# peterzjx/DeepHall

Hardware: AMD Instinct MI355X
Metric: local-energies/sec + MCMC walker-steps/sec, N=6 2Q=15, 1/2/4/8 GPUs (higher is better)
Workload: dtype f32; 1 GPU; VMC iteration (mcmc_step 10 MH moves + local energy + stats all-reduce), nspins=[6, 0] flux=15, Psiformer 4x64 heads, 2 layers, 1 det; walkers_per_gpu=4096, global_batch=4096, parallelism=walker-dp1, walker_groups_per_gpu=1, gemm_arithmetic=x6all

## Files before the change

### deephall_amd/_lib.py

```python

from __future__ import annotations

import ctypes as C
import os
from pathlib import Path

LIB_PATH = Path(__file__).resolve().parent / "_lib" / "libdeephall_amd.so"

DH_NSTATS = 16
STAT_NAMES = [
    "energy_re",
    "energy_im",
    "clipped_re",
    "clipped_im",
    "ere2",
    "kinetic_re",
    "kinetic_im",
    "potential",
    "angular_momentum_z",
    "angular_momentum_z_square",
    "angular_momentum_square",
    "pmove",
    "nvalid",
    "clipped_lz2",
    "clipped_lz",
    "clipped_l2",
]

EXPORTS = [
    "dh_create",
    "dh_create_cf",
    "dh_destroy",
    "dh_last_error",
    "dh_version",
    "dh_param_layout",
    "dh_set_params",
    "dh_workspace_bytes",
    "dh_set_gemm_mode",
    "dh_logpsi",
    "dh_mcmc_step",
    "dh_local_energy",
    "dh_energy_stats",
    "dh_loss_diff",
    "dh_init_walkers",
    "dh_potential",
    "dh_histograms",
    "dh_monopole_orbitals",
    "dh_mh_init",
    "dh_mh_propose",
    "dh_mh_accept",
    "dh_kinetic_from_derivatives",
    "dh_debug_trunk",
    "dh_debug_gemm",
    "dh_debug_gemm_ln",
    "dh_debug_gemm_x6_ln",
    "dh_debug_chain_x6",
    "dh_debug_gemm_lnch",
    "dh_debug_set_lnch_form",
    "dh_debug_x6_plane_rows",
    "dh_debug_split_planes",
    "dh_debug_gemm_x6",
    "dh_debug_gemm_x6_choice",
    "dh_debug_route",
    "dh_ref_layout",
    "dh_set_params_ref",
    "dh_vjp_workspace_bytes",
    "dh_logpsi_vjp",
    "dh_grad_cotangent",
    "dh_adam_update",
    "dh_profile_enable",
    "dh_profile_read",
    "dh_debug_f_offset",
    "dh_debug_env_leaf",
    "dh_kfac_layout",
    "dh_kfac_workspace_bytes",
    "dh_kfac_vjp",
    "dh_kfac_step",
    "dh_ntk_workspace_bytes",
    "dh_ntk_tile_walkers",
    "dh_ntk",
    "dh_ntk_part",
    "dh_ntk_mirror",
    "dh_ntk_owner",
    "dh_minsr_matrix_workspace_bytes",
    "dh_minsr_matrix",
    "dh_ntk_jvp_workspace_bytes",
    "dh_ntk_jvp",
    "dh_fidelity_partial",
    "dh_fidelity_residual",
]

DH_NFID = 5


PROF_KINDS = ["gemm", "attention", "layernorm", "input", "det_value", "det_energy", "mcmc",
              "gemm_ch", "attention_ch", "layernorm_ch", "input_ch", "layer1_ch"]


class DhConfig(C.Structure):
    _fields_ = [
        ("struct_size", C.c_uint32),
        ("n_up", C.c_int),
        ("n_dn", C.c_int),
        ("flux", C.c_int),
        ("radius", C.c_float),
        ("interaction_strength", C.c_float),
        ("interaction_type", C.c_int),
        ("num_heads", C.c_int),
        ("heads_dim", C.c_int),
        ("num_layers", C.c_int),
        ("ndets", C.c_int),
        ("orbital_type", C.c_int),
        ("network_type", C.c_int),
        ("excitation_lz", C.c_float),
        ("cf_flux", C.c_int),
    ]

    def __init__(self, *args, **kw):
        super().__init__(*args, **kw)
        self.struct_size = C.sizeof(DhConfig)


_lib = None


def load(path: Path | str | None = None):
    global _lib
    if _lib is not None:
        return _lib
    p = Path(path) if path else Path(os.environ.get("DH_LIB_PATH") or LIB_PATH)
    if not p.exists():
        raise RuntimeError(
            f"deephall_amd HIP library not found at {p}. Build it with "
            "`python -c 'import __graft_entry__ as g; g.build()'` (no CPU fallback exists)."
        )
    lib = C.CDLL(str(p))
    vp, sz, i32, u64, i64 = C.c_void_p, C.c_size_t, C.c_int, C.c_uint64, C.c_int64
    lib.dh_create.argtypes = [C.POINTER(DhConfig), C.POINTER(vp)]
    lib.dh_create.restype = i32
    lib.dh_create_cf.argtypes = [C.POINTER(DhConfig), C.POINTER(C.c_int), i32, C.POINTER(vp)]
    lib.dh_create_cf.restype = i32
    lib.dh_destroy.argtypes = [vp]
    lib.dh_destroy.restype = None
    lib.dh_last_error.restype = C.c_char_p
    lib.dh_version.restype = C.c_char_p
    lib.dh_param_layout.argtypes = [vp, C.POINTER(sz), i32]
    lib.dh_param_layout.restype = i32
    lib.dh_set_params.argtypes = [vp, vp, sz, vp]
    lib.dh_set_params.restype = i32
    lib.dh_workspace_bytes.argtypes = [vp, i32, i32]
    lib.dh_workspace_bytes.restype = sz
    lib.dh_set_gemm_mode.argtypes = [vp, i32]
    lib.dh_set_gemm_mode.restype = i32
    lib.dh_logpsi.argtypes = [vp, vp, i32, vp, vp, sz, vp]
    lib.dh_logpsi.restype = i32
    lib.dh_mcmc_step.argtypes = [vp, vp, vp, vp, i32, i32, C.c_float, u64, u64, i64, vp, vp, sz, vp]
    lib.dh_mcmc_step.restype = i32
    lib.dh_local_energy.argtypes = [vp, vp, i32, vp, vp, vp, sz, vp]
    lib.dh_local_energy.restype = i32
    lib.dh_energy_stats.argtypes = [vp, vp, vp, vp, i32, i32, i32, vp, vp]
    lib.dh_energy_stats.restype = i32
    f32 = C.c_float
    lib.dh_loss_diff.argtypes = [vp, vp, vp, i32, vp, f32, f32, f32, vp, vp, vp]
    lib.dh_loss_diff.restype = i32
    lib.dh_init_walkers.argtypes = [vp, vp, i32, u64, i64, vp]
    lib.dh_init_walkers.restype = i32
    lib.dh_potential.argtypes = [vp, vp, i32, vp, vp]
    lib.dh_potential.restype = i32
    lib.dh_histograms.argtypes = [vp, i32, i32, i32, i32, vp, vp, vp]
    lib.dh_histograms.restype = i32
    lib.dh_monopole_orbitals.argtypes = [vp, i32, i32, vp, vp]
    lib.dh_monopole_orbitals.restype = i32
    lib.dh_debug_trunk.argtypes = [vp, vp, i32, i32, vp, sz, vp]
    lib.dh_debug_trunk.restype = i32
    lib.dh_debug_f_offset.argtypes = [vp, i32, i32]
    lib.dh_debug_f_offset.restype = sz
    lib.dh_debug_env_leaf.argtypes = [vp, i32, i32, i32, vp, vp]
    lib.dh_debug_env_leaf.restype = i32
    lib.dh_debug_gemm.argtypes = [i32, vp, i32, vp, i32, vp, vp, i32, vp, i32, i32, i32, i32, i32, vp]
    lib.dh_debug_gemm.restype = i32
    lib.dh_debug_gemm_ln.argtypes = [i32, i32, vp, i32, vp, i32, vp, vp, vp, i32, i32, vp]
    lib.dh_debug_gemm_ln.restype = i32
    lib.dh_debug_gemm_x6_ln.argtypes = [i32, i32, vp, i32, vp, i32, vp, vp, vp, i32, i32, vp]
    lib.dh_debug_gemm_x6_ln.restype = i32
    lib.dh_debug_chain_x6.argtypes = [vp, vp, i32, vp, vp, vp, i32, vp, vp, vp, i32, vp, i32, vp, i32, vp, i32, vp]
    lib.dh_debug_chain_x6.restype = i32
    lib.dh_debug_gemm_lnch.argtypes = [i32, i32, vp, vp, i32, vp, vp, vp, vp, i32, vp]
    lib.dh_debug_gemm_lnch.restype = i32
    lib.dh_debug_set_lnch_form.argtypes = [i32]
    lib.dh_debug_set_lnch_form.restype = i32
    lib.dh_debug_x6_plane_rows.argtypes = [i32]
    lib.dh_debug_x6_plane_rows.restype = i32
    lib.dh_debug_split_planes.argtypes = [vp, i32, i32, i32, vp, vp]
    lib.dh_debug_split_planes.restype = i32
    lib.dh_debug_gemm_x6.argtypes = [i32, vp, i32, vp, i32, vp, vp, i32, vp, i32, i32, i32, i32, i32, vp]
    lib.dh_debug_gemm_x6.restype = i32
    lib.dh_debug_gemm_x6_choice.argtypes = [i32, i32]
    lib.dh_debug_gemm_x6_choice.restype = i32
    lib.dh_debug_route.argtypes = [vp, i32, i32, C.POINTER(i32), i32]
    lib.dh_debug_route.restype = i32
    lib.dh_ref_layout.argtypes = [vp, C.POINTER(sz), i32]
    lib.dh_ref_layout.restype = i32
    lib.dh_set_params_ref.argtypes = [vp, vp, sz, vp]
    lib.dh_set_params_ref.restype = i32
    lib.dh_vjp_workspace_bytes.argtypes = [vp, i32]
    lib.dh_vjp_workspace_bytes.restype = sz
    lib.dh_logpsi_vjp.argtypes = [vp, vp, i32, vp, vp, vp, vp, sz, vp]
    lib.dh_logpsi_vjp.restype = i32
    lib.dh_kfac_layout.argtypes = [vp, C.POINTER(sz), i32]
    lib.dh_kfac_layout.restype = i32
    lib.dh_kfac_workspace_bytes.argtypes = [vp, i32]
    lib.dh_kfac_workspace_bytes.restype = sz
    lib.dh_kfac_vjp.argtypes = [vp, vp, i32, vp, vp, vp, vp, vp, sz, vp]
    lib.dh_kfac_vjp.restype = i32
    lib.dh_kfac_step.argtypes = [vp, vp, vp, f32, f32, vp, vp, f32, f32, f32, vp, vp, vp, sz, vp]
    lib.dh_kfac_step.restype = i32
    lib.dh_ntk_workspace_bytes.argtypes = [vp, i32]
    lib.dh_ntk_workspace_bytes.restype = sz
    lib.dh_ntk_tile_walkers.argtypes = [vp]
    lib.dh_ntk_tile_walkers.restype = i32
    lib.dh_ntk.argtypes = [vp, vp, i32, vp, vp, vp, vp, sz, vp]
    lib.dh_ntk.restype = i32
    lib.dh_ntk_part.argtypes = [vp, vp, i32, vp, vp, vp, vp, sz, i32, i32, vp]
    lib.dh_ntk_part.restype = i32
    lib.dh_ntk_mirror.argtypes = [vp, i32, vp]
    lib.dh_ntk_mirror.restype = i32
    lib.dh_ntk_owner.argtypes = [vp, i32, i32]
    lib.dh_ntk_owner.restype = i32
    lib.dh_minsr_matrix_workspace_bytes.argtypes = [i32]
    lib.dh_minsr_matrix_workspace_bytes.restype = sz
    lib.dh_minsr_matrix.argtypes = [vp, vp, i32, C.c_double, vp, vp, sz, vp]
    lib.dh_minsr_matrix.restype = i32
    lib.dh_ntk_jvp_workspace_bytes.argtypes = [vp, i32]
    lib.dh_ntk_jvp_workspace_bytes.restype = sz
    lib.dh_ntk_jvp.argtypes = [vp, vp, i32, vp, vp, vp, vp, vp, vp, sz, i32, i32, vp]
    lib.dh_ntk_jvp.restype = i32
    lib.dh_fidelity_partial.argtypes = [vp, vp, i32, vp, vp]
    lib.dh_fidelity_partial.restype = i32
    lib.dh_fidelity_residual.argtypes = [vp, vp, i32, vp, vp, vp]
    lib.dh_fidelity_residual.restype = i32
    lib.dh_grad_cotangent.argtypes = [vp, vp, i32, i32, vp, vp]
    lib.dh_grad_cotangent.restype = i32
    lib.dh_adam_update.argtypes = [vp, vp, vp, vp, sz, f32, f32, f32, f32, i32, vp]
    lib.dh_adam_update.restype = i32
    lib.dh_mh_init.argtypes = [vp, vp, vp, i32, vp]
    lib.dh_mh_init.restype = i32
    lib.dh_mh_propose.argtypes = [vp, vp, i32, i32, f32, u64, u64, i64, vp, vp]
    lib.dh_mh_propose.restype = i32
    lib.dh_mh_accept.argtypes = [vp, vp, vp, vp, vp, i32, i32, u64, u64, i64, vp, vp]
    lib.dh_mh_accept.restype = i32
    lib.dh_kinetic_from_derivatives.argtypes = [vp, vp, vp, i32, i32, C.c_double, C.c_double, vp, vp, vp]
    lib.dh_kinetic_from_derivatives.restype = i32
    lib.dh_profile_enable.argtypes = [vp, i32]
    lib.dh_profile_enable.restype = i32
    lib.dh_profile_read.argtypes = [vp, C.POINTER(C.c_double), i32]
    lib.dh_profile_read.restype = i32
    _lib = lib
    return lib


def check(rc: int):
    if rc != 0:
        msg = load().dh_last_error().decode(errors="replace")
        raise RuntimeError(f"deephall_amd error {rc}: {msg}")
```

### deephall_amd/csrc/api.cpp

```cpp
#include <hip/hip_runtime.h>

#include <cmath>
#include <cstdio>
#include <cstring>
#include <string>
#include <vector>

#include "dh_internal.h"

using namespace dh;

namespace {
thread_local std::string g_err;

int fail(int code, const std::string& msg) {
  g_err = msg;
  return code;
}

#define HIP_TRY(expr)                                                                       \
  do {                                                                                      \
    hipError_t e_ = (expr);                                                                 \
    if (e_ != hipSuccess) return fail(DH_EHIP, std::string(#expr ": ") + hipGetErrorString(e_)); \
  } while (0)
// ... 661 lines not shown
  launch_copy2d(ref(R.jas(0)), 1, pk(so + 2), 1, 1, 1, st);
  launch_copy2d(ref(R.jas(1)), 1, pk(so + 2) + 1, 1, 1, 1, st);
  if (d.L > 0) launch_small_gemm(4, 3 * D, D, pk(0), D, 0, pk(1), 3 * D, 0, pk(so + 3), 3 * D, 0, st);
}

}

extern "C" {

int dh_set_params(dh_handle* h, const float* params, size_t count, void* stream) {
  if (h && h->analytic()) return count == 0 ? DH_OK : fail(DH_EINVAL, "the Laughlin wavefunction has no parameters");
  if (!h || !params) return fail(DH_EINVAL, "null argument");
  if (count != h->offsets.back()) return fail(DH_EINVAL, "parameter count mismatch");
  if (int rc = ensure_param_buffers(h)) return rc;
  HIP_TRY(hipMemcpyAsync(h->params, params, count * sizeof(float), hipMemcpyDeviceToDevice, (hipStream_t)stream));
  assign_packed(h);
  if (int rc = derive_weights(h, (hipStream_t)stream)) return rc;
  h->params_set = true;
  h->ref_set = false;
  return DH_OK;
}

int dh_ref_layout(const dh_handle* h, size_t* offsets, int n) {
  if (!h) return fail(DH_EINVAL, "null handle");
  const int nseg = (int)h->ref_offsets.size() - 1;
  for (int i = 0; i < n && i <= nseg; ++i) offsets[i] = h->ref_offsets[i];
  return nseg;
}

int dh_set_params_ref(dh_handle* h, const float* ref, size_t count, void* stream) {
  if (h && h->analytic()) return count == 0 ? DH_OK : fail(DH_EINVAL, "the Laughlin wavefunction has no parameters");
  if (!h || !ref) return fail(DH_EINVAL, "null argument");
  if (count != h->ref_offsets.back()) return fail(DH_EINVAL, "reference parameter count mismatch");
  if (int rc = ensure_param_buffers(h)) return rc;
  if (!h->ref) HIP_TRY(hipMalloc(&h->ref, count * sizeof(float)));
  hipStream_t st = (hipStream_t)stream;
  HIP_TRY(hipMemcpyAsync(h->ref, ref, count * sizeof(float), hipMemcpyDeviceToDevice, st));
  pack_from_ref(h, st);
  HIP_TRY(hipGetLastError());
  assign_packed(h);
  if (int rc = derive_weights(h, st)) return rc;
  h->params_set = true;
  h->ref_set = true;
  return DH_OK;
}

int dh_set_gemm_mode(dh_handle* h, int mode) {
  if (!h) return fail(DH_EINVAL, "null handle");
  if (mode != DH_GEMM_F32 && mode != DH_GEMM_X6 && mode != DH_GEMM_X6_ALL && mode != DH_GEMM_X6_ALL_UNFUSED)
    return fail(DH_EINVAL, "bad GEMM mode");
  h->gemm_mode = mode;
  return DH_OK;
}

size_t dh_workspace_bytes(const dh_handle* h, int batch, int op) {
  if (!h || batch < 1) return 0;
  return carve(h->d, h->gemm_mode, batch, op == 1 ? h->d.C : 1, nullptr).total_bytes;
}

}

namespace {

void dense_gemm(int family, const float* X, int ldx, const float* W, const float* Wt, const uint16_t* Wp, int ldw,
                const float* bias, const float* Res, int ldr, float* Y, int ldy, int rows, int ncols, int K, int C,
                hipStream_t s) {
  if (family == GEMM_X6)
    launch_gemm_x6(X, ldx, Wp, x6_plane_rows(ncols), bias, Res, ldr, Y, ldy, rows, ncols, K, C, s);
  else if (family == GEMM_F32_NT)
    launch_gemm_nt(X, ldx, Wt, K, bias, Res, ldr, Y, ldy, rows, ncols, K, C, s);
  else
    launch_gemm(X, ldx, W, ldw, bias, Res, ldr, Y, ldy, rows, ncols, K, C, s);
}

struct Trunk {
  dh_handle* h;
  const Dims& d;
  const Params& P;
  const Work& w;
  hipStream_t s;
  const int nw, C, rows;
  const TrunkRoute r;
  const bool keep_h;
  const int D = d.D, KO = ofeat_k(d);
  const int ch = C > 1 ? PK_CH : 0;
  const double R = rows, DD = D, f4 = 4.0;

  void gemm(const float* X, int ldx, const float* W, const float* Wt, const uint16_t* Wp, int ldw, const float* bias,
            const float* Res, int ldr, float* Y, int ldy, int ncols, int K) const {
    PROF(PK_GEMM + ch, 2.0 * R * ncols * K, f4 * (R * K + (double)K * ncols + R * ncols * (Res ? 2 : 1)));
    dense_gemm(r.family, X, ldx, W, Wt, Wp, ldw, bias, Res, ldr, Y, ldy, rows, ncols, K, C, s);
  }
  X6Feat h0_feat(int l) const { return (r.h0_epilogue && l == 0) ? X6Feat{P.W0, w.geo, d.N, d.n_up} : X6Feat{}; }

  void layer_chain(int l, bool attn) const {
    const LayerParams& lp = P.layer[l];
    const bool last = l + 1 == d.L;
    const int n3 = last ? d.orb_cols : 3 * D;
    PROF(PK_GEMM, 2.0 * R * DD * (2.0 * DD + n3), f4 * (2.0 * R * DD + R * n3 + 2.0 * DD * DD + DD * n3));
    X6Feat feat = h0_feat(l);
    if (attn) {
      feat.W0qkv = P.W0qkv;
      feat.bqkv = lp.bqkv;
      feat.Mqk = P.Mqk;
      feat.L1V = P.L1VP;
      feat.L1B = P.L1BP;
    }
    launch_chain_x6(w.o, attn ? P.UP : lp.WolP, x6_plane_rows(D), lp.bol, lp.ln1, lp.WmP, x6_plane_rows(D), lp.bm,
                    lp.ln2, last ? P.WorbP : P.layer[l + 1].WqkvP, x6_plane_rows(n3),
                    last ? P.borb : P.layer[l + 1].bqkv, n3, last ? w.F : w.qkv, last ? d.ld_orb : 3 * D, w.h, rows,
                    feat, s, !last || keep_h);
  }
  void layer_ln_epilogue(int l) const {
    const LayerParams& lp = P.layer[l];
    const bool x6 = r.family == GEMM_X6;
    {
      PROF(PK_GEMM, 2.0 * R * DD * DD, f4 * (3.0 * R * DD + DD * DD));
      if (x6)
        launch_gemm_x6_ln(w.o, D, lp.WolP, x6_plane_rows(D), lp.bol, lp.ln1, w.h, rows, D, 0, 0, s, h0_feat(l));
      else
        launch_gemm_ln(w.o, D, lp.WolT, D, lp.bol, lp.ln1, w.h, rows, D, 0, 0, s);
    }
    PROF(PK_GEMM, 2.0 * R * DD * DD, f4 * (2.0 * R * DD + DD * DD));
    if (x6)
      launch_gemm_x6_ln(w.h, D, lp.WmP, x6_plane_rows(D), lp.bm, lp.ln2, w.h, rows, D, 1, 0, s);
    else
      launch_gemm_ln(w.h, D, lp.WmT, D, lp.bm, lp.ln2, w.h, rows, D, 1, 0, s);
  }
  void layer_lnch(int l) const {
    const LayerParams& lp = P.layer[l];
    {
      const bool of = r.ofeat && l == 0;
      const double KK = of ? KO : DD;
      PROF(PK_GEMM + PK_CH, 2.0 * R * DD * KK, f4 * (R * KK + 2.0 * R * DD + DD * KK));
      launch_gemm_lnch(d.N, w.o, of ? P.UP : lp.WolP, x6_plane_rows(D), lp.bol, lp.ln1, w.geo, w.h, nw * d.N, 0, s,
                       (r.h0_epilogue && l == 0) ? P.W0 : nullptr, d.n_up, of ? KO : D);
    }
    PROF(PK_GEMM + PK_CH, 2.0 * R * DD * DD, f4 * (3.0 * R * DD + DD * DD));
    launch_gemm_lnch(d.N, w.h, lp.WmP, x6_plane_rows(D), lp.bm, lp.ln2, w.geo, w.h, nw * d.N, 1, s);
  }
  void layer_lnch_whole() const {
    const LayerParams& lp = P.layer[0];
    PROF(PK_L1CH, 2.0 * R * DD * 3.0 * KO, f4 * (R * KO + R * DD));
    launch_gemm_lnch(d.N, w.o, P.UP, x6_plane_rows(D), lp.bol, lp.ln2, w.geo, w.h, nw * d.N, 2, s, P.W0, d.n_up, KO,
                     P.L1VP, P.L1BP);
  }
  void layer_l1ch() const {
    const LayerParams& lp = P.layer[0];
    PROF(PK_L1CH, 2.0 * R * DD * (24.0 + 27.0), f4 * (R * KO + R * DD));
    launch_layer1_ch(d, w.o, P.UT, P.L1VT, P.W0, lp.bol, lp.ln1, lp.ln2, w.geo, w.h, nw, s);
  }
  void layer_separate(int l) const {
    const LayerParams& lp = P.layer[l];
    const bool lf = r.h0_epilogue && l == 0;
    if (r.ofeat && l == 0)
      gemm(w.o, KO, nullptr, P.UT, P.UP, KO, lp.bol, lf ? nullptr : w.h, D, w.t, D, D, KO);
    else
      gemm(w.o, D, lp.Wol, lp.WolT, lp.WolP, D, lp.bol, lf ? nullptr : w.h, D, w.t, D, D, D);
    {
      PROF(PK_LN + ch, 0.0, f4 * R * 2.0 * DD);
      launch_layernorm(d, w.t, nullptr, lp.ln1, w.geo, w.h, nw, C, 0, s, lf ? P.W0 : nullptr);
    }
    gemm(w.h, D, lp.Wm, lp.WmT, lp.WmP, D, lp.bm, nullptr, 0, w.o, D, D, D);
    PROF(PK_LN + ch, 0.0, f4 * R * 3.0 * DD);
    launch_layernorm(d, nullptr, w.o, lp.ln2, w.geo, w.h, nw, C, 1, s);
  }

  int run(const float* x, bool geo_ready) const {
    if (!(geo_ready && r.input_skip)) {
      const bool wq = r.input_qkv;
      PROF(PK_INPUT + ch, 8.0 * R * DD * (wq ? 4 : 1), f4 * R * DD * (wq ? 4 : 1));
      launch_input(d, x, P.W0, wq ? P.W0qkv : nullptr, wq ? P.layer[0].bqkv : nullptr, r.input_h ? w.h : nullptr,
                   wq ? w.qkv : nullptr, w.geo, nw, C, s);
    }
    for (int l = 0; l < d.L; ++l) {
      const LayerParams& lp = P.layer[l];
      const int form = l == 0 ? r.form0 : r.form1;
      if (l > 0 && r.qkv_gemm)
        gemm(w.h, D, lp.Wqkv, lp.WqkvT, lp.WqkvP, 3 * D, lp.bqkv, nullptr, 0, w.qkv, 3 * D, 3 * D, D);
      if (form != LF_CHAIN_ATTN) {
        const bool f = r.attn_feat && l == 0;
        PROF(PK_ATTN + ch, 0.0, f4 * R * (f ? 1.0 : 4.0) * DD);
        launch_attention(d, w.qkv, w.geo, w.o, nw, C, s, f ? P.W0qkv : nullptr, f ? lp.bqkv : nullptr,
                         f ? P.Mqk : nullptr);
      }
      switch (form) {
        case LF_CHAIN:
        case LF_CHAIN_ATTN: layer_chain(l, form == LF_CHAIN_ATTN); break;
        case LF_LN_EPILOGUE: layer_ln_epilogue(l); break;
        case LF_LNCH_WHOLE: layer_lnch_whole(); break;
        case LF_LNCH_PAIR: layer_lnch(l); break;
        case LF_L1CH: layer_l1ch(); break;
        default: layer_separate(l); break;
      }
    }
    if (r.orbital == ORB_GEMM)
      gemm(w.h, D, P.Worb, P.WorbT, P.WorbP, d.ld_orb, P.borb, nullptr, 0, w.F, d.ld_orb, d.orb_cols, D);
    return check_launch();
  }
};

int run_trunk(dh_handle* h, const float* x, int nw, int C, const Work& w, hipStream_t s, bool geo_ready = false,
              bool keep_h = false) {
  return Trunk{h, h->d, h->p, w, s, nw, C, nw * h->d.N * C, w.route, keep_h}.run(x, geo_ready);
}

int launch_trial(dh_handle* h, const float* x, float* logpsi, float* e_l, float* obs, int nw, hipStream_t s) {
  if (!h->expo && !h->expo_host.empty()) {
    HIP_TRY(hipMalloc(&h->expo, h->expo_host.size() * sizeof(int)));
    HIP_TRY(hipMemcpy(h->expo, h->expo_host.data(), h->expo_host.size() * sizeof(int), hipMemcpyHostToDevice));
  }
  PROF(e_l ? PK_DET_ENERGY : PK_DET_VALUE, 0.0, e_l ? 48.0 * nw : 8.0 * nw * h->d.N);
  if (h->state == dh_handle::PFAFFIAN)
    launch_pfaffian(h->d, x, h->cfg.cf_flux, logpsi, e_l, obs, nw, s);
  else if (h->state == dh_handle::JAIN)
    launch_cf(h->d, x, h->expo, h->cf_dense, logpsi, e_l, obs, nw, s);
  else
    launch_laughlin(h->d, x, h->expo, logpsi, e_l, obs, nw, s);
  return check_launch();
}

int value_pass(dh_handle* h, const float* x, int nw, const Work& w, float* logpsi, hipStream_t s,
               bool geo_ready = false, const McmcEpi& epi = McmcEpi{}) {
  if (h->analytic()) return launch_trial(h, x, logpsi, nullptr, nullptr, nw, s);
  if (int rc = run_trunk(h, x, nw, 1, w, s, geo_ready)) return rc;
  {
    PROF(PK_DET_VALUE, 0.0, 4.0 * nw * h->d.N * h->d.ld_orb);
    launch_det_value(h->d, w.F, x, h->p.jastrow, h->norm, logpsi, nw, s, epi);
  }
  return check_launch();
}

int check_common(dh_handle* h, const void* x, int B, void* ws, size_t ws_bytes, size_t need) {
  if (!h) return fail(DH_EINVAL, "null handle");
  if (!h->params_set) return fail(DH_ESTATE, "parameters not set");
  if (!x || B < 1) return fail(DH_EINVAL, "bad walkers");
  if (!ws || ws_bytes < need) return fail(DH_ENOMEM, "workspace too small");
  return DH_OK;
}

}

extern "C" {

int dh_logpsi(dh_handle* h, const float* x, int B, float* logpsi, void* ws, size_t ws_bytes, void* stream) {
  const size_t need = h ? dh_workspace_bytes(h, B, 0) : 0;
  if (int rc = check_common(h, x, B, ws, ws_bytes, need)) return rc;
  if (!logpsi) return fail(DH_EINVAL, "null output");
  hipStream_t s = (hipStream_t)stream;
  Work w = carve(h->d, h->gemm_mode, B, 1, ws);
  return value_pass(h, x, B, w, logpsi, s);
}

int dh_mcmc_step(dh_handle* h, float* x, float* lp, int32_t* n_accept, int B, int steps, float width, uint64_t seed,
                 uint64_t counter, int64_t walker_offset, const float* noise, void* ws, size_t ws_bytes,
                 void* stream) {
  const size_t need = h ? dh_workspace_bytes(h, B, 0) : 0;
  if (int rc = check_common(h, x, B, ws, ws_bytes, need)) return rc;
  if (!lp || !n_accept || steps < 0) return fail(DH_EINVAL, "bad MCMC arguments");
  hipStream_t s = (hipStream_t)stream;
  const Dims& d = h->d;
  Work w = carve(d, h->gemm_mode, B, 1, ws);
  if (int rc = value_pass(h, x, B, w, w.logpsi, s)) return rc;
  launch_lp_from_logpsi(w.logpsi, lp, n_accept, B, s);
  const size_t nstride = (size_t)B * (2 * d.N + 1);
  const bool geo = !h->analytic();
  const bool fuse = geo;
  for (int st = 0; st < steps; ++st) {
    const float* nz = noise ? noise + st * nstride : nullptr;
    const uint64_t step = counter + (uint64_t)st;
    if (!fuse || st == 0) {
      PROF(PK_MCMC, 0.0, 16.0 * B * d.N);
      if (st == 0)
        launch_propose(d, x, w.x2, B, width, seed, step, walker_offset, nz, 0, s, geo ? w.geo : nullptr);
      else
        launch_accept_propose(d, x, w.x2, geo ? w.geo : nullptr, lp, w.logpsi, n_accept, B, width, seed, step - 1,
                              walker_offset, noise ? noise + (st - 1) * nstride : nullptr, nz, s);
    }
    McmcEpi epi{};
    if (fuse) {
      epi.on = 1;
      epi.propose = st + 1 < steps;
      epi.x = x;
      epi.x2 = w.x2;
      epi.geo = w.geo;
      epi.lp = lp;
      epi.nacc = n_accept;
      epi.width = width;
      epi.seed = seed;
      epi.step = step;
      epi.woff = walker_offset;
      epi.noise = nz;
      epi.noise2 = (noise && st + 1 < steps) ? noise + (st + 1) * nstride : nullptr;
    }
    if (int rc = value_pass(h, w.x2, B, w, w.logpsi, s, geo, epi)) return rc;
  }
  if (steps > 0 && !fuse) {
    PROF(PK_MCMC, 0.0, 16.0 * B * d.N);
    launch_accept(d, x, w.x2, lp, w.logpsi, n_accept, B, seed, counter + (uint64_t)(steps - 1), walker_offset,
                  noise ? noise + (steps - 1) * nstride : nullptr, 0, s);
  }
  return check_launch();
}

int dh_local_energy(dh_handle* h, const float* x, int B, float* e_l, float* obs, void* ws, size_t ws_bytes,
                    void* stream) {
  const size_t need1 = h ? dh_workspace_bytes(h, 1, 1) : 0;
// ... 785 lines not shown
    launch_small_gemm(D + 1, D, D + 1, stats + K.slots[L.A_o].off, D + 1, 0, Wt, D, 0, T, D, 0, s);
    launch_small_gemm(D, D, D + 1, Wt, D, 1, T, D, 0, stats + K.slots[L.A_Wl].off, D, 0, s);
    launch_small_gemm(D, D, D, ref(RS.lay(l, RWl)), D, 0, stats + K.slots[L.G_T].off, D, 0, T, D, 0, s);
    launch_small_gemm(D, D, D, T, D, 0, ref(RS.lay(l, RWl)), D, 1, stats + K.slots[L.G_out].off, D, 0, s);
  }
  launch_kfac_generic(w.fgrad, K.dev.gen, stats + K.nmat, 1.f / (float)B, s);
  return check_launch();
}

int dh_kfac_step(dh_handle* h, float* raw, const float* stats, float ema, float weight, const float* grad,
                 float* params, float lr, float damping, float norm_constraint, float* pgrad, double* info, void* ws,
                 size_t ws_bytes, void* stream) {
  if (!h || h->analytic()) return fail(DH_EINVAL, "KFAC needs a Psiformer handle");
  if (!raw || !grad || !pgrad || !info || !ws) return fail(DH_EINVAL, "null argument");
  if (!(weight > 0.f) || !(damping > 0.f)) return fail(DH_EINVAL, "KFAC needs weight > 0 and damping > 0");
  if (int rc = kfac_device(h)) return rc;
  const KfacHost& K = *h->kfac;
  const size_t nref = h->ref_offsets.back();
  if (ws_bytes < kfac_step_ws(&K)) return fail(DH_ENOMEM, "KFAC step workspace too small");
  hipStream_t s = (hipStream_t)stream;
  double* kbuf = reinterpret_cast<double*>(ws);
  double* tr = kbuf + align64(K.kbuf_doubles);
  double* tmp = tr + align64(K.slots.size());
  if (stats) launch_kfac_ema(raw, stats, K.nstats, ema, s);
  launch_kfac_invert(K.dev, raw, 1.0 / weight, std::sqrt((double)damping), tr, kbuf, tmp, s);
  launch_kfac_precondition(K.dev, grad, raw + K.nmat, 1.0 / weight, damping, kbuf, pgrad, nref, info, s);
  if (params) launch_kfac_update(params, pgrad, nref, info, lr, norm_constraint, s);
  return check_launch();
}

int dh_grad_cotangent(const float* diff, const float* nvalid, int B, int part, float* ct, void* stream) {
  if (!diff || !nvalid || !ct || B < 1 || (part != 0 && part != 1)) return fail(DH_EINVAL, "bad arguments");
  launch_cotangent(diff, nvalid, B, part, ct, (hipStream_t)stream);
  return check_launch();
}

int dh_adam_update(float* params, const float* grad, float* mu, float* nu, size_t n, float lr, float b1, float b2,
                   float eps, int step, void* stream) {
  if (!params || !grad || !mu || !nu || n == 0 || step < 0) return fail(DH_EINVAL, "bad arguments");
  launch_adam(params, grad, mu, nu, n, lr, b1, b2, eps, step, (hipStream_t)stream);
  return check_launch();
}

int dh_energy_stats(dh_handle* h, const float* e_l, const float* obs, const int32_t* n_accept, int B, int steps,
                    int penalties, float* out, void* stream) {
  (void)h;
  if (!e_l || !obs || !out) return fail(DH_EINVAL, "null argument");
  if (B < 1) return fail(DH_EINVAL, "dh_energy_stats needs B >= 1");
  launch_stats(e_l, obs, n_accept, B, steps, penalties, out, (hipStream_t)stream);
  return check_launch();
}

int dh_loss_diff(dh_handle* h, const float* e_l, const float* obs, int B, const float* stats, float lz_penalty,
                 float lz_center, float l2_penalty, float* diff, float* nvalid, void* stream) {
  (void)h;
  if (!e_l || !obs || !stats || !diff || !nvalid) return fail(DH_EINVAL, "null argument");
  if (B < 1) return fail(DH_EINVAL, "dh_loss_diff needs B >= 1");
  launch_loss_diff(e_l, obs, B, stats, lz_penalty, lz_center, l2_penalty, diff, nvalid, (hipStream_t)stream);
  return check_launch();
}

int dh_fidelity_partial(const float* logpsi, const float* logphi, int B, double* part, void* stream) {
  if (!logpsi || !logphi || !part) return fail(DH_EINVAL, "dh_fidelity_partial: null argument");
  if (B < 1) return fail(DH_EINVAL, "dh_fidelity_partial needs B >= 1");
  launch_fidelity_partial(logpsi, logphi, B, part, (hipStream_t)stream);
  return check_launch();
}

int dh_fidelity_residual(const float* logpsi, const float* logphi, int B, const double* total, float* resid,
                         void* stream) {
  if (!logpsi || !logphi || !total || !resid) return fail(DH_EINVAL, "dh_fidelity_residual: null argument");
  if (B < 1) return fail(DH_EINVAL, "dh_fidelity_residual needs B >= 1");
  launch_fidelity_residual(logpsi, logphi, B, total, resid, (hipStream_t)stream);
  return check_launch();
}

int dh_debug_trunk(dh_handle* h, const float* x, int B, int op, void* ws, size_t ws_bytes, void* stream) {
  const size_t need = h ? dh_workspace_bytes(h, B, op) : 0;
  if (int rc = check_common(h, x, B, ws, ws_bytes, need)) return rc;
  Work w = carve(h->d, h->gemm_mode, B, op == 1 ? h->d.C : 1, ws);
  if (!w.F)
    return fail(DH_EINVAL, "dh_debug_trunk: this config's local energy goes envelope first and maps no orbital "
                           "features F over the channel rows");
  return run_trunk(h, x, B, op == 1 ? h->d.C : 1, w, (hipStream_t)stream, false, true);
}

int dh_debug_env_leaf(const float* thph, int n, int M, int sq, float* out, void* stream) {
  if (!thph || !out || n < 1 || M < 1) return fail(DH_EINVAL, "bad env_leaf probe args");
  launch_env_leaf_probe(thph, n, M, sq, out, (hipStream_t)stream);
  return check_launch();
}

size_t dh_debug_f_offset(const dh_handle* h, int B, int op) {
  if (!h || B < 1) return (size_t)-1;
  Work w = carve(h->d, h->gemm_mode, B, op == 1 ? h->d.C : 1, reinterpret_cast<void*>(size_t(64)));
  if (!w.F) return (size_t)-1;
  return (size_t)(w.F - reinterpret_cast<float*>(size_t(64)));
}

int dh_debug_gemm(int variant, const float* X, int ldx, const float* W, int ldw, const float* bias, const float* R,
                  int ldr, float* Y, int ldy, int rows, int ncols, int K, int C, void* stream) {
  bool known = true;
  if (variant >= 100) {
    if (K % 32 != 0) return fail(DH_EINVAL, "NT GEMM needs K % 32 == 0");
    known = launch_gemm_nt_variant(variant - 100, X, ldx, W, ldw, bias, R, ldr, Y, ldy, rows, ncols, K, C,
                                   (hipStream_t)stream);
  } else {
    known = launch_gemm_variant(variant < 0 ? 0 : variant, X, ldx, W, ldw, bias, R, ldr, Y, ldy, rows, ncols, K, C,
                                (hipStream_t)stream);
  }
  if (!known) return fail(DH_EINVAL, "no GEMM variant " + std::to_string(variant));
  return check_launch();
}

int dh_debug_gemm_x6_choice(int rows, int ncols) { return gemm_x6_choose(rows, ncols); }

int dh_debug_route(const dh_handle* h, int B, int op, int* out, int n) {
  if (!h || h->analytic() || B < 1 || (n > 0 && !out)) return fail(DH_EINVAL, "bad route query");
  const int C = op == 1 ? h->d.C : 1;
  const TrunkRoute r = trunk_route(h->d, h->gemm_mode, C, B * h->d.N * C);
  if (n > 0) std::memcpy(out, &r, sizeof(int) * std::min(n, kTrunkRouteFields));
  return kTrunkRouteFields;
}

int dh_debug_x6_plane_rows(int ncols) { return x6_plane_rows(ncols); }

int dh_debug_split_planes(const float* Wt, int ldw, int ncols, int K, uint16_t* Wp, void* stream) {
  if (!Wt || !Wp || ncols < 1 || K < 1) return fail(DH_EINVAL, "bad split_planes args");
  launch_split_planes(Wt, ldw, ncols, K, Wp, (hipStream_t)stream);
  return check_launch();
}

int dh_debug_gemm_x6(int variant, const float* X, int ldx, const uint16_t* Wp, int ldp, const float* bias,
                     const float* R, int ldr, float* Y, int ldy, int rows, int ncols, int K, int C, void* stream) {
  if (!gemm_x6_supported(K) || ldp < x6_plane_rows(ncols)) return fail(DH_EINVAL, "bad gemm_x6 args");
  if (variant >= 10 && K > 256) return fail(DH_EINVAL, "persistent gemm_x6 needs K <= 256");
  if (variant < 0) variant = gemm_x6_choose(rows, ncols);
  if (!launch_gemm_x6_variant(variant, X, ldx, Wp, ldp, bias, R, ldr, Y, ldy, rows, ncols, K, C, (hipStream_t)stream))
    return fail(DH_EINVAL, "no gemm_x6 variant " + std::to_string(variant));
  return check_launch();
}

int dh_debug_gemm_x6_ln(int mode, int nw, const float* X, int ldx, const uint16_t* Wp, int ldp, const float* bias,
                        const float* ln, float* h, int rows, int K, void* stream) {
  if (!gemm_x6_supported(K) || K > 256 || ldp < x6_plane_rows(256) || rows < 1 || (mode != 0 && mode != 1))
    return fail(DH_EINVAL, "bad gemm_x6_ln args");
  if (!launch_gemm_x6_ln(X, ldx, Wp, ldp, bias, ln, h, rows, K, mode, nw, (hipStream_t)stream))
    return fail(DH_EINVAL, "no gemm_x6_ln form " + std::to_string(nw));
  return check_launch();
}

int dh_debug_chain_x6(const float* X1, const uint16_t* Wp1, int ldp1, const float* b1, const float* ln1,
                      const uint16_t* Wp2, int ldp2, const float* b2, const float* ln2, const uint16_t* Wp3,
                      int ldp3, const float* b3, int n3, float* Y3, int ldy3, float* h, int rows, void* stream) {
  if (!X1 || !Wp1 || !Wp2 || !b1 || !ln1 || !b2 || !ln2 || !h || rows < 1 || ldp1 < x6_plane_rows(256) ||
      ldp2 < x6_plane_rows(256) || (Wp3 && (!b3 || !Y3 || n3 < 1 || ldy3 < n3 || ldy3 % 4 || ldp3 < x6_plane_rows(n3))))
    return fail(DH_EINVAL, "bad chain_x6 args");
  launch_chain_x6(X1, Wp1, ldp1, b1, ln1, Wp2, ldp2, b2, ln2, Wp3, ldp3, b3, n3, Y3, ldy3, h, rows, X6Feat{},
                  (hipStream_t)stream);
  return check_launch();
}

int dh_debug_gemm_lnch(int N, int mode, const float* X, const uint16_t* Wp, int ldp, const float* bias,
                       const float* ln, const float* geo, float* h, int ne, void* stream) {
  if (!gemm_lnch_supported(N, 256) || (mode != 0 && mode != 1) || (mode == 0 && !X) || !Wp || !ln || !geo || !h ||
      ne < 1 || ldp < x6_plane_rows(256) || ne % N)
    return fail(DH_EINVAL, "bad gemm_lnch args");
  launch_gemm_lnch(N, mode == 0 ? X : h, Wp, ldp, bias, ln, geo, h, ne, mode, (hipStream_t)stream);
  return check_launch();
}

int dh_debug_set_lnch_form(int form) { return set_lnch_form(form); }

int dh_debug_gemm_ln(int mode, int bm, const float* X, int ldx, const float* Wt, int ldw, const float* bias,
                     const float* ln, float* h, int rows, int K, void* stream) {
  if (!gemm_ln_supported(256, K) || rows < 1 || (mode != 0 && mode != 1)) return fail(DH_EINVAL, "bad gemm_ln args");
  launch_gemm_ln(X, ldx, Wt, ldw, bias, ln, h, rows, K, mode, bm, (hipStream_t)stream);
  return check_launch();
}

int dh_profile_enable(dh_handle* h, int on) {
  if (!h) return fail(DH_EINVAL, "null handle");
  h->prof.on = on != 0;
  h->prof.used = 0;
  return DH_OK;
}

int dh_profile_read(dh_handle* h, double* out, int reset) {
  if (!h || !out) return fail(DH_EINVAL, "null argument");
  for (int i = 0; i < 4 * PK_TOTAL; ++i) out[i] = 0.0;
  for (size_t i = 0; i < h->prof.used; ++i) {
    ProfRec& r = h->prof.recs[i];
    HIP_TRY(hipEventSynchronize(r.b));
    float ms = 0.f;
    HIP_TRY(hipEventElapsedTime(&ms, r.a, r.b));
    out[4 * r.kind + 0] += 1.0;
    out[4 * r.kind + 1] += ms;
    out[4 * r.kind + 2] += r.flops;
    out[4 * r.kind + 3] += r.bytes;
  }
  if (reset) h->prof.used = 0;
  return PK_TOTAL;
}

int dh_potential(dh_handle* h, const float* x, int B, float* pe, void* stream) {
  if (!h || !x || !pe || B < 1) return fail(DH_EINVAL, "bad arguments");
  launch_potential(h->d, x, pe, B, (hipStream_t)stream);
  return check_launch();
}

int dh_histograms(const float* x, int B, int nelec, int density_bins, int pair_bins, float* density, float* pair,
                  void* stream) {
  if (!x || B < 1 || nelec < 1 || density_bins < 0 || pair_bins < 0 || density_bins + pair_bins < 1 ||
      density_bins + pair_bins > 8192 || (density_bins && !density) || (pair_bins && !pair))
    return fail(DH_EINVAL, "bad arguments");
  launch_histograms(x, B, nelec, density_bins, pair_bins, density, pair, (hipStream_t)stream);
  return check_launch();
}

int dh_monopole_orbitals(const float* points, int n, int flux, float* out, void* stream) {
  if (!points || !out || n < 1 || flux < 0 || flux > 126) return fail(DH_EINVAL, "bad arguments");
  launch_monopole_orbitals(points, n, flux, out, (hipStream_t)stream);
  return check_launch();
}


int dh_mh_init(const float* logpsi, float* lp, int32_t* n_accept, int B, void* stream) {
  if (!logpsi || !lp || !n_accept || B < 1) return fail(DH_EINVAL, "bad arguments");
  launch_lp_from_logpsi(logpsi, lp, n_accept, B, (hipStream_t)stream);
  return check_launch();
}

int dh_mh_propose(const float* x, float* x2, int B, int nelec, float width, uint64_t seed, uint64_t step,
                  int64_t walker_offset, const float* noise, void* stream) {
  if (!x || !x2 || B < 1 || nelec < 1 || x == x2) return fail(DH_EINVAL, "bad arguments");
  Dims d{};
  d.N = nelec;
  launch_propose(d, x, x2, B, width, seed, step, walker_offset, noise, 0, (hipStream_t)stream);
  return check_launch();
}

int dh_mh_accept(float* x, const float* x2, float* lp, const float* logpsi2, int32_t* n_accept, int B, int nelec,
                 uint64_t seed, uint64_t step, int64_t walker_offset, const float* noise, void* stream) {
  if (!x || !x2 || !lp || !logpsi2 || !n_accept || B < 1 || nelec < 1) return fail(DH_EINVAL, "bad arguments");
  Dims d{};
  d.N = nelec;
  launch_accept(d, x, x2, lp, logpsi2, n_accept, B, seed, step, walker_offset, noise, 0, (hipStream_t)stream);
  return check_launch();
}

int dh_kinetic_from_derivatives(const double* x, const double* grad, const double* hess, int B, int nelec, double Q,
                                double r, float* ke, float* mom, void* stream) {
  if (!x || !grad || !hess || !ke || !mom || B < 1 || nelec < 1 || !(r > 0.0) || Q < 0.0)
    return fail(DH_EINVAL, "bad arguments");
  if (kinetic_assembly_lds_bytes(nelec) > 64 * 1024) return fail(DH_EINVAL, "nelec > 256");
// ... 12 lines not shown
```

### deephall_amd/csrc/det.hip

```cpp
#include <cstdlib>
#include <type_traits>

#include "dh_internal.h"
#include "device_common.h"
#include "mcmc_common.h"

#ifndef DET_LU_REG
#define DET_LU_REG 0
#endif
#ifndef DET_WAVE_SQ
#define DET_WAVE_SQ 1
#endif
#ifndef DET_LEAF_SQ
#define DET_LEAF_SQ 1
#endif
#ifndef DET_GJ_REG
#define DET_GJ_REG 1
#endif
#ifndef DET_STAMP
#define DET_STAMP 0
#endif
#if DET_STAMP
constexpr int DET_STAMP_WG = 1024, DET_NSTAMP = 12;
__device__ unsigned long long g_det_stamp[2 * DET_STAMP_WG * DET_NSTAMP];
#define DET_T(slot, i)                                                                                       \
  do {                                                                                                      \
    if (threadIdx.x == 0 && blockIdx.x < DET_STAMP_WG)                                                       \
      g_det_stamp[((slot) * DET_STAMP_WG + blockIdx.x) * DET_NSTAMP + (i)] = __builtin_amdgcn_s_memtime();     \
  } while (0)
extern "C" int dh_debug_det_stamps(unsigned long long* out, int n) {
  n = n < 2 * DET_STAMP_WG * DET_NSTAMP ? n : 2 * DET_STAMP_WG * DET_NSTAMP;
  return hipMemcpyFromSymbol(out, HIP_SYMBOL(g_det_stamp), n * sizeof(unsigned long long)) == hipSuccess ? 0 : -1;
}
#else
#define DET_T(slot, i)
#endif

namespace dh {
namespace {

__device__ inline float ipow(float b, int e) { return e < 0 ? 0.f : (e == 0 ? 1.f : powf(b, (float)e)); }
__device__ inline float ipow_sq(float b, int e) {
  float r = 1.f;
  for (; e > 0; e >>= 1, b *= b)
    if (e & 1) r *= b;
  return r;
}

struct FView {
  const float* F;
  int ld, M, N, K;
  __device__ inline cf at(size_t row, int blk, int m, int j, int k) const {
    const size_t base = row * ld;
    const int MNK = M * N * K;
    const int off = m * N * K + j * K + k;
    return cf{F[base + (size_t)(blk * 2) * MNK + off], F[base + (size_t)(blk * 2 + 1) * MNK + off]};
  }
};

struct EnvLeaf {
  cf e0, dth, dph, lb, d2th;
};
__device__ __forceinline__ float env_gauge(float ct, int M) {
  return (float)(M - 1) * __builtin_rintf(64.f * ct) * (1.f / 128.f);
}
__device__ inline EnvLeaf env_leaf(float th, float ph, int p, int M, float norm, bool leaves, float gauge = 0.f,
                                   bool sq = false) {
  const int a = p, b = M - 1 - p;
  const float m = 0.5f * (float)(a - b) - gauge;
  float c, s;
  sincosf(0.5f * th, &s, &c);
  float sph, cph;
  sincosf(m * ph, &sph, &cph);
  const float R = sq ? ipow_sq(c, a) * ipow_sq(s, b) : ipow(c, a) * ipow(s, b);
  EnvLeaf L;
  L.e0 = cf{norm * R * cph, norm * R * sph};
  if (leaves) {
    const float fa = (float)a, fb = (float)b;
    auto pw = [sq](float x, int e) { return sq ? (e < 0 ? 0.f : ipow_sq(x, e)) : ipow(x, e); };
    const float R1 = 0.5f * (fb * pw(c, a + 1) * pw(s, b - 1) - fa * pw(c, a - 1) * pw(s, b + 1));
    const float R2 = 0.25f * (fb * (fb - 1.f) * pw(c, a + 2) * pw(s, b - 2) - fb * (fa + 1.f) * R -
                              fa * (fb + 1.f) * R + fa * (fa - 1.f) * pw(c, a - 2) * pw(s, b + 2));
    float st, ct;
    sincosf(th, &st, &ct);
    L.dth = cf{norm * R1 * cph, norm * R1 * sph};
    L.d2th = cf{norm * R2 * cph, norm * R2 * sph};
    L.dph = cf{-m * L.e0.im / st, m * L.e0.re / st};
    const float cot = ct / st;
    const float k2 = m * m / (st * st);
    L.lb = cf{L.d2th.re - k2 * L.e0.re + cot * L.dth.re, L.d2th.im - k2 * L.e0.im + cot * L.dth.im};
  }
  return L;
}

__device__ inline cf env_flow2(const cf& e0, const cf& dth, const cf& d2th, float m, float st, float ct, float sp,
                               float cp, int k) {
  const float cot = ct / st;
  const float ph_hat[3] = {-sp, cp, 0.f};
  const float th_hat[3] = {ct * cp, ct * sp, -st};
  const float thp[3] = {cp * cot, sp * cot, -1.f};
  const float dthp_dth[3] = {-cp / (st * st), -sp / (st * st), 0.f};
  const float dthp_dph[3] = {-sp * cot, cp * cot, 0.f};
  const float cs[3] = {cp, sp, 0.f};
  const float td = ph_hat[k];
  const float pd = -th_hat[k] / st;
  const float tdd = cs[k] * thp[k];
  const float pdd = -(dthp_dth[k] * td - dthp_dph[k] * thp[k]);
  cf r;
  r.re = d2th.re * td * td + 2.f * (-m * dth.im) * td * pd + (-m * m * e0.re) * pd * pd + dth.re * tdd +
         (-m * e0.im) * pdd;
  r.im = d2th.im * td * td + 2.f * (m * dth.re) * td * pd + (-m * m * e0.im) * pd * pd + dth.im * tdd +
         (m * e0.re) * pdd;
  return r;
}

__device__ inline void find_pivot(const cf* A, int lda, int N, int p, int* piv, int tid, int width) {
  if (tid < width) {
    const int lane = tid;
    float best = -1.f;
    int bi = N;
    for (int r = p + lane; r < N; r += width) {
      const float v = cabs1(A[r * lda + p]);
      if (v > best) {
        best = v;
        bi = r;
      }
    }
    for (int o = width >> 1; o > 0; o >>= 1) {
      const float ob = __shfl_xor(best, o, width);
      const int oi = __shfl_xor(bi, o, width);
      if (ob > best || (ob == best && oi < bi)) {
        best = ob;
        bi = oi;
      }
    }
    if (lane == 0) *piv = (bi < N) ? bi : p;
  }
}

__device__ __forceinline__ void eliminate(cf* A, int lda, int N, int ncol, bool gj, cf* fac, int* piv, cf* logdet,
                          int tid = threadIdx.x, int nt = blockDim.x, int width = 64) {
  if (tid == 0) *logdet = cf{0.f, 0.f};
  __syncthreads();
  for (int p = 0; p < N; ++p) {
    find_pivot(A, lda, N, p, piv, tid, width);
    __syncthreads();
    const int pr = *piv;
    if (pr != p) {
      for (int c = tid; c < ncol; c += nt) {
        const cf t = A[p * lda + c];
        A[p * lda + c] = A[pr * lda + c];
        A[pr * lda + c] = t;
      }
    }
    __syncthreads();
    const cf P = A[p * lda + p];
    if (tid == 0) {
      const float mag = sqrtf(P.re * P.re + P.im * P.im);
      logdet->re += logf(mag);
      logdet->im += atan2f(P.im, P.re) + (pr != p ? kPi : 0.f);
    }
    const cf Pinv = cdiv(cf{1.f, 0.f}, P);
    __syncthreads();
    if (gj) {
      for (int r = tid; r < N; r += nt) fac[r] = (r == p) ? cf{0.f, 0.f} : A[r * lda + p];
      for (int c = tid; c < ncol; c += nt) A[p * lda + c] = A[p * lda + c] * Pinv;
    } else {
      for (int r = tid; r < N; r += nt) fac[r] = (r > p) ? A[r * lda + p] * Pinv : cf{0.f, 0.f};
    }
    __syncthreads();
    const int r0 = gj ? 0 : p + 1;
    const int c0 = gj ? 0 : p;
    const int nr = N - r0, nc = ncol - c0;
    for (int idx = tid; idx < nr * nc; idx += nt) {
      const int r = r0 + idx / nc, c = c0 + idx % nc;
      if (r == p) continue;
      const cf f = fac[r];
      cf v = A[r * lda + c];
      const cf a = A[p * lda + c];
      v.re -= f.re * a.re - f.im * a.im;
      v.im -= f.re * a.im + f.im * a.re;
      A[r * lda + c] = v;
    }
    __syncthreads();
  }
}

template <int NMAX>
__device__ __forceinline__ cf gj_inverse_cols(cf (&col)[NMAX], int N) {
  auto is = [](int r, int q) __attribute__((always_inline)) {
    int m = r == q;
    asm volatile("" : "+v"(m));
    return m != 0;
  };
  auto pick = [&](int q) __attribute__((always_inline)) {
    cf v = col[0];
#pragma unroll
    for (int r = 1; r < NMAX; ++r)
      if (is(r, q)) v = col[r];
    return v;
  };
  float lre = 0.f, lim = 0.f;
  for (int p = 0; p < N; ++p) {
    float best = -1.f;
    int bi = N;
#pragma unroll
    for (int r = 0; r < NMAX; ++r) {
      if (r >= p && r < N) {
        const float v = cabs1(col[r]);
        if (v > best) {
          best = v;
          bi = r;
        }
      }
    }
    int pr = __shfl(bi, p, 64);
    pr = pr < N ? pr : p;
    if (pr != p) {
      const cf a = pick(p), b = pick(pr);
#pragma unroll
      for (int r = 0; r < NMAX; ++r) {
        if (is(r, p)) col[r] = b;
        if (is(r, pr)) col[r] = a;
      }
    }
    const cf mine = pick(p);
    const cf P{__shfl(mine.re, p, 64), __shfl(mine.im, p, 64)};
    const float mag = sqrtf(P.re * P.re + P.im * P.im);
    lre += logf(mag);
    lim += atan2f(P.im, P.re) + (pr != p ? kPi : 0.f);
    const cf rowp = mine * cdiv(cf{1.f, 0.f}, P);
#pragma unroll
    for (int r = 0; r < NMAX; ++r) {
      if (r < N) {
        const cf f{__shfl(col[r].re, p, 64), __shfl(col[r].im, p, 64)};
        cf v = col[r];
        v.re -= f.re * rowp.re - f.im * rowp.im;
        v.im -= f.re * rowp.im + f.im * rowp.re;
        col[r] = is(r, p) ? rowp : v;
      }
    }
  }
  return cf{lre, lim};
}

template <int NMAX>
__device__ __forceinline__ cf lu_logdet_cols(cf (&col)[NMAX], int N, int lane, int width) {
  auto is = [](int r, int q) __attribute__((always_inline)) {
    int m = r == q;
    asm volatile("" : "+v"(m));
    return m != 0;
  };
  auto pick = [&](int q) __attribute__((always_inline)) {
    cf v = col[0];
#pragma unroll
    for (int r = 1; r < NMAX; ++r)
      if (is(r, q)) v = col[r];
    return v;
  };
  float lre = 0.f, lim = 0.f;
  for (int p = 0; p < N; ++p) {
    float best = -1.f;
    int bi = N;
#pragma unroll
    for (int r = 0; r < NMAX; ++r) {
      if (r >= p && r < N) {
        const float v = cabs1(col[r]);
        if (v > best) {
          best = v;
          bi = r;
        }
      }
    }
    int pr = __shfl(bi, p, width);
    pr = pr < N ? pr : p;
    if (pr != p) {
      const cf a = pick(p), b = pick(pr);
#pragma unroll
      for (int r = 0; r < NMAX; ++r) {
        if (is(r, p)) col[r] = b;
        if (is(r, pr)) col[r] = a;
      }
    }
    const cf mine = pick(p);
    const cf P{__shfl(mine.re, p, width), __shfl(mine.im, p, width)};
    const float mag = sqrtf(P.re * P.re + P.im * P.im);
    lre += logf(mag);
    lim += atan2f(P.im, P.re) + (pr != p ? kPi : 0.f);
    const cf Pinv = cdiv(cf{1.f, 0.f}, P);
#pragma unroll
    for (int r = 0; r < NMAX; ++r) {
      if (r > p && r < N) {
#pragma clang fp contract(off)
        const cf c = col[r];
        const cf fl{c.re * Pinv.re - c.im * Pinv.im, __builtin_fmaf(c.im, Pinv.re, c.re * Pinv.im)};
        const cf f{__shfl(fl.re, p, width), __shfl(fl.im, p, width)};
        if (lane >= p) {
          const float tre = __builtin_fmaf(f.re, mine.re, -(f.im * mine.im));
          const float tim = __builtin_fmaf(f.im, mine.re, f.re * mine.im);
          col[r] = cf{c.re - tre, c.im - tim};
        }
      }
    }
  }
  return cf{lre, lim};
}

__device__ inline double jastrow_pair(double r, double al, double cst, double* f1, double* f2) {
  const double ar = al + r;
  *f1 = (cst * al * al) / (ar * ar);
  *f2 = -2.0 * (cst * al * al) / (ar * ar * ar);
  return -(cst * al * al) / ar;
}

template <int MGV, bool HW = false>
__global__ __launch_bounds__(64) void det_value_kernel(const float* __restrict__ Fp, int ldF, const float* x,
                                 const float* __restrict__ jas, const float* __restrict__ norm, float* __restrict__ logpsi,
                                 int N, int n_up, int M, int K, int nw, int per, McmcEpi epi) {
  static_assert(!HW || MGV == 0, "half-wave form: serial contraction only");
  extern __shared__ float sm_all[];
  const int half = HW ? (int)(threadIdx.x >> 5) : 0;
  float* sm_raw = sm_all + half * per;
  cf* E0 = reinterpret_cast<cf*>(sm_raw);
  cf* A = E0 + N * M;
  cf* fac = A + N * N;
  cf* ld = fac + N;
  cf* logdet = ld + K;
  int* piv = reinterpret_cast<int*>(logdet + 1);
  const int bw = HW ? 2 * (int)blockIdx.x + half : (int)blockIdx.x;
  const bool live = bw < nw;
  const int b = live ? bw : nw - 1;
  const int tid = HW ? (int)(threadIdx.x & 31) : (int)threadIdx.x, nt = HW ? 32 : 64, width = HW ? 32 : 64;
  double* cart = reinterpret_cast<double*>(piv + 2);
  DET_T(0, 0);
  for (int idx = tid; idx < N * M; idx += nt) {
    const int i = idx / M, p = idx % M;
    E0[idx] = env_leaf(x[2 * (b * N + i)], x[2 * (b * N + i) + 1], p, M, norm[p], false, 0.f, true).e0;
  }
  for (int i = tid; i < N; i += nt) {
    double st, ct, sp, cp;
    sincos((double)x[2 * (b * N + i)], &st, &ct);
    sincos((double)x[2 * (b * N + i) + 1], &sp, &cp);
    cart[3 * i] = st * cp;
    cart[3 * i + 1] = st * sp;
    cart[3 * i + 2] = ct;
  }
  __syncthreads();
  DET_T(0, 1);
  double Jw = 0.0;
  {
    const double ap = jas[0], aa = jas[1];
    for (int q = tid; q < N * N; q += nt) {
      const int i = q / N, j = q - (q / N) * N;
      if (j <= i) continue;
      const double dx = cart[3 * j] - cart[3 * i], dy = cart[3 * j + 1] - cart[3 * i + 1],
                   dz = cart[3 * j + 2] - cart[3 * i + 2];
      const double r = sqrt(dx * dx + dy * dy + dz * dz);
      const bool same = (i < n_up) == (j < n_up);
      double f1, f2;
      Jw += jastrow_pair(r, same ? ap : aa, same ? 0.25 : 0.5, &f1, &f2);
    }
    for (int o = width >> 1; o > 0; o >>= 1) Jw += __shfl_xor(Jw, o, width);
  }
  DET_T(0, 2);
  const int G = 64 / N, gj = tid % N, gg = tid / N, NK = N * K, MNK = M * NK;
  for (int k = 0; k < K; ++k) {
    if constexpr (MGV == 0) {
      for (int idx = tid; idx < N * N; idx += nt) {
        const int i = idx / N, j = idx % N;
        const int blk = (i >= n_up && n_up > 0) ? 1 : 0;
        const float* rp = Fp + ((size_t)b * N + i) * ldF + (size_t)blk * 2 * MNK + (size_t)j * K + k;
        cf acc{0.f, 0.f};
        for (int p0 = 0; p0 < M; p0 += 16) {
          float fr[16], fi[16];
#pragma unroll
          for (int q = 0; q < 16; ++q) {
            const size_t p = (size_t)min(p0 + q, M - 1);
            fr[q] = rp[p * NK];
            fi[q] = rp[(size_t)MNK + p * NK];
          }
#pragma unroll
          for (int q = 0; q < 16; ++q)
            if (p0 + q < M) cfma(acc, cf{fr[q], fi[q]}, E0[i * M + p0 + q]);
        }
        A[idx] = acc;
      }
    }
    if constexpr (MGV > 0) {
      constexpr int NF = 2 * (MGV > 0 ? MGV : 1);
      auto ldrow = [&](int i, float (&f)[NF]) __attribute__((always_inline)) {
        const int blk = (i >= n_up && n_up > 0) ? 1 : 0;
        const float* rp = Fp + ((size_t)b * N + i) * ldF + (size_t)blk * 2 * MNK + (size_t)gj * K + k;
#pragma unroll
        for (int u = 0; u < MGV; ++u) {
          const size_t m = (size_t)min(gg + G * u, M - 1);
          f[2 * u] = rp[m * NK];
          f[2 * u + 1] = rp[(size_t)MNK + m * NK];
        }
      };
      auto contract = [&](int i, const float (&f)[NF]) __attribute__((always_inline)) {
        cf acc{0.f, 0.f};
#pragma unroll
        for (int u = 0; u < MGV; ++u) {
          const int m = gg + G * u;
          const bool ok = gg < G && m < M;
          cfma(acc, cf{ok ? f[2 * u] : 0.f, ok ? f[2 * u + 1] : 0.f}, E0[i * M + min(m, M - 1)]);
        }
        float re = acc.re, im = acc.im;
        for (int q = 1; q < G; ++q) {
          re += __shfl(acc.re, gj + N * q, 64);
          im += __shfl(acc.im, gj + N * q, 64);
        }
        if (gg == 0) A[i * N + gj] = cf{re, im};
      };
      float fa[NF], fb[NF];
      if constexpr (MGV <= 24) {
        ldrow(0, fa);
        for (int i = 0; i < N; i += 2) {
          ldrow(min(i + 1, N - 1), fb);
          contract(i, fa);
          ldrow(min(i + 2, N - 1), fa);
          if (i + 1 < N) contract(i + 1, fb);
        }
      } else {
        for (int i = 0; i < N; ++i) {
          ldrow(i, fa);
          contract(i, fa);
        }
      }
    }
    __syncthreads();
    DET_T(0, 3);
    if (N <= 8 && DET_LU_REG) {
      cf col[8];
#pragma unroll
      for (int r = 0; r < 8; ++r) col[r] = (r < N && tid < N) ? A[r * N + tid] : cf{0.f, 0.f};
      const cf l = lu_logdet_cols<8>(col, N, tid, width);
      if (tid == 0) ld[k] = l;
    } else {
      eliminate(A, N, N, N, false, fac, piv, logdet, tid, nt, width);
      if (tid == 0) ld[k] = *logdet;
    }
    __syncthreads();
    DET_T(0, 4);
  }
  float* lpv = reinterpret_cast<float*>(cart + 3 * N);
  if (tid == 0 && live) {
    float lmax = -INFINITY;
    for (int k = 0; k < K; ++k) lmax = fmaxf(lmax, ld[k].re);
    float zr = 0.f, zi = 0.f;
    for (int k = 0; k < K; ++k) {
      const float mag = expf(ld[k].re - lmax);
      zr += mag * cosf(ld[k].im);
      zi += mag * sinf(ld[k].im);
    }
    float val_re = 0.5f * logf(zr * zr + zi * zi) + lmax;
    float val_im = atan2f(zi, zr);
    logpsi[2 * b] = val_re + (float)Jw;
    logpsi[2 * b + 1] = val_im;
    *lpv = val_re + (float)Jw;
  }
  DET_T(0, 5);
  if (!epi.on) return;
  __syncthreads();
  if (!live || tid >= N) return;
  const float lp2 = 2.f * *lpv;
  const bool cond = accept_one(lp2, epi.lp[b], b, N, epi.seed, epi.step, epi.woff, epi.noise);
  const int e = b * N + tid;
  float th = epi.x[2 * e], ph = epi.x[2 * e + 1];
  if (cond) {
    th = x[2 * e];
    ph = x[2 * e + 1];
    epi.x[2 * e] = th;
    epi.x[2 * e + 1] = ph;
    if (tid == 0) {
      epi.lp[b] = lp2;
      epi.nacc[b] += 1;
    }
  }
  if (epi.propose)
    propose_one(th, ph, epi.x2, epi.geo, e, b, tid, N, epi.width, epi.seed, epi.step + 1, epi.woff, epi.noise2);
  DET_T(0, 6);
}

#ifndef ENV_REG
#define ENV_REG 1
#endif
#ifndef ENV_SEG_RING
#define ENV_SEG_RING 4
#endif
constexpr int kEnvSegRing = ENV_SEG_RING;
__host__ __device__ constexpr int env_ring(int MG) { return (63 / (2 * MG) + 1) < 4 ? (63 / (2 * MG) + 1) : 4; }

template <int MG, bool WU = false, int SEG = 0>
__global__ __launch_bounds__(256) void env_contract_kernel(const float* __restrict__ Fp, int ldF,
                                                           const float* __restrict__ x,
                                                           const float* __restrict__ geo_g,
                                                           const float* __restrict__ norm, float* __restrict__ PhiC,
                                                           int nw, int N, int n_up, int M, int K, float Q) {
  static_assert(SEG == 0 || !WU, "segment DMA: four waves per electron");
  constexpr int Q2 = SEG ? 2 * SEG : 2 * MG, RING = SEG ? kEnvSegRing : env_ring(MG);
  static_assert((RING - 1) * Q2 <= 63, "vmcnt range");
  extern __shared__ float sm[];
  const int tid = threadIdx.x, lane = tid & 63, wv = tid >> 6;
  const int unit = WU ? blockIdx.x * 4 + wv : blockIdx.x;
  if (WU && unit >= nw * N) return;
  const int b = unit / N, i = unit - (unit / N) * N;
  const int T = 2 * N, C = 2 * N + 5;
  const int wsz = WU ? 20 * M + ((3 * T + 3) & ~3) + RING * Q2 * 64 : 0;
  cf* wt = reinterpret_cast<cf*>(sm + (size_t)wv * wsz);
  cf* part = wt + 10 * M;
  float* al = reinterpret_cast<float*>(WU ? part : part + 4 * C * N);
  float* ring = al + ((3 * T + 3) & ~3);
  const int G = 64 / N, j = lane % N, g = lane / N, S = WU ? G : 4 * G;
  const int MW = (M + 3) / 4;
  const int gg = SEG ? MW * wv + g : (WU ? g : G * wv + g);
  const int mend = SEG ? min(MW * (wv + 1), M) : M;
  const bool act = g < G;
  const int blk = (i >= n_up && n_up > 0) ? 1 : 0;
  const int NK = N * K, MNK = M * NK;
  auto gsum = [&](float v) __attribute__((always_inline)) {
    float r = v;
    for (int q = 1; q < G; ++q) r += __shfl(v, j + N * q, 64);
    return r;
  };
  auto gsumc = [&](cf v) __attribute__((always_inline)) { return cf{gsum(v.re), gsum(v.im)}; };
  const float* rowbase = Fp + ((size_t)(b * N + i) * C) * ldF + (size_t)blk * 2 * MNK + (size_t)j * K;
  const int SS = SEG ? G : S;
  auto mw = [&](int u) __attribute__((always_inline)) { return min(gg + SS * u, M - 1); };
  auto okm = [&](int u) __attribute__((always_inline)) { return act && gg + SS * u < mend; };
  const int segf = MW * N * K;
  float* wring = WU ? ring : ring + (size_t)wv * RING * (SEG ? 2 * segf : Q2 * 64);
  const uint32_t ring0 = (uint32_t)(size_t)((__attribute__((address_space(3))) char*)wring);
  const float* segbase = Fp + ((size_t)(b * N + i) * C) * ldF + (size_t)blk * 2 * MNK + (size_t)MW * wv * NK;
  const int segb = (mend - MW * wv) * NK * 4;
  auto issue = [&](int c, int kd) __attribute__((always_inline)) {
    if constexpr (SEG > 0) {
      (void)kd;
      const int slot = c % RING;
#pragma unroll
      for (int q = 0; q < 2 * SEG; ++q) {
        const int p = q / SEG, piece = q % SEG;
        const int byte = piece * 1024 + lane * 16;
        const char* src = reinterpret_cast<const char*>(segbase + (size_t)c * ldF + (p ? (size_t)MNK : 0)) + byte;
        const uint32_t dst = __builtin_amdgcn_readfirstlane(ring0 + (uint32_t)(slot * 2 * segf * 4 + p * segf * 4 + piece * 1024));
        if (byte < segb) {
          unsigned keep;
          asm volatile("s_mov_b32 %0, m0\n\ts_mov_b32 m0, %2\n\ts_nop 0\n\tglobal_load_lds_dwordx4 %1, off\n\ts_mov_b32 m0, %0"
                       : "=&s"(keep)
                       : "v"(src), "s"(dst)
                       : "memory");
        }
      }
      return;
    }
    const float* rp = rowbase + (size_t)c * ldF + kd;
    const int slot = c % RING;
#pragma unroll
    for (int q = 0; q < Q2; ++q) {
      const int u = q >> 1;
      const float* src = okm(u) ? rp + ((q & 1) ? (size_t)MNK : 0) + (size_t)(gg + S * u) * NK : rowbase;
      const uint32_t dst = __builtin_amdgcn_readfirstlane(ring0 + (uint32_t)((slot * Q2 + q) * 256));
      unsigned keep;
      asm volatile("s_mov_b32 %0, m0\n\ts_mov_b32 m0, %2\n\ts_nop 0\n\tglobal_load_lds_dword %1, off\n\ts_mov_b32 m0, %0"
                   : "=&s"(keep)
// ... 1343 lines not shown
      const int blk = (i >= n_up && n_up > 0) ? 1 : 0;
      const size_t row = (size_t)b * N + i;
      cf acc{0.f, 0.f};
      for (int p = 0; p < M; ++p) cfma(acc, F.at(row, blk, p, j, k), E0[i * M + p]);
      A[i * lda + j] = acc;
      if (lda > N) A[i * lda + N + j] = cf{i == j ? 1.f : 0.f, 0.f};
    }
    __syncthreads();
  };
  if (K > 1) {
    for (int k = 0; k < K; ++k) {
      build(k, N);
      eliminate(A, N, N, N, false, fac, piv, logdet);
      if (tid == 0) ld[k] = *logdet;
      __syncthreads();
    }
    if (tid == 0) {
      float lmax = -INFINITY;
      for (int k = 0; k < K; ++k) lmax = fmaxf(lmax, ld[k].re);
      cf z{0.f, 0.f};
      for (int k = 0; k < K; ++k) {
        const float mag = expf(ld[k].re - lmax);
        z += cf{mag * cosf(ld[k].im), mag * sinf(ld[k].im)};
      }
      for (int k = 0; k < K; ++k) {
        const float mag = expf(ld[k].re - lmax);
        wk[k] = cdiv(cf{mag * cosf(ld[k].im), mag * sinf(ld[k].im)}, z);
      }
    }
  } else if (tid == 0) {
    wk[0] = cf{1.f, 0.f};
  }
  __syncthreads();
  for (int k = 0; k < K; ++k) {
    build(k, 2 * N);
    eliminate(A, 2 * N, N, 2 * N, true, fac, piv, logdet);
    const cf w = wk[k];
    for (int idx = tid; idx < N * M * N; idx += nt) {
      const int i = idx / (M * N), rem = idx - i * (M * N), p = rem / N, j = rem - (rem / N) * N;
      const int blk = (i >= n_up && n_up > 0) ? 1 : 0;
      const cf f = w * A[j * 2 * N + N + i];
      const cf G{cr * f.re + ci * f.im, ci * f.re - cr * f.im};
      const cf e = E0[i * M + p];
      const cf v{G.re * e.re + G.im * e.im, G.im * e.re - G.re * e.im};
      const size_t rowoff = ((size_t)b * N + i) * ldF;
      const int off = p * N * K + j * K + k;
      dF[rowoff + (size_t)(blk * 2) * MNK + off] = v.re;
      dF[rowoff + (size_t)(blk * 2 + 1) * MNK + off] = v.im;
    }
    __syncthreads();
  }
}

__global__ void potential_kernel(const float* __restrict__ x, float* __restrict__ pe, int nw, int N, float Q,
                                 float radius, int interaction) {
  const int b = blockIdx.x * blockDim.x + threadIdx.x;
  if (b >= nw) return;
  double acc = 0.0;
  for (int i = 0; i < N; ++i) {
    const double ti = x[2 * (b * N + i)], pi_ = x[2 * (b * N + i) + 1];
    const double xi = sin(ti) * cos(pi_), yi = sin(ti) * sin(pi_), zi = cos(ti);
    for (int j = i + 1; j < N; ++j) {
      const double tj = x[2 * (b * N + j)], pj = x[2 * (b * N + j) + 1];
      const double u = xi * sin(tj) * cos(pj) + yi * sin(tj) * sin(pj) + zi * cos(tj);
      if (interaction == DH_INTERACTION_COULOMB)
        acc += 1.0 / sqrt(2.0 - 2.0 * u);
      else
        acc += 1.0 + ((double)Q + 1.0) / (double)Q * u;
    }
  }
  if (interaction == DH_INTERACTION_COULOMB) acc /= (double)radius;
  pe[b] = (float)acc;
}

}

void launch_potential(const Dims& d, const float* x, float* pe, int nw, hipStream_t s) {
  hipLaunchKernelGGL(potential_kernel, dim3((nw + 127) / 128), dim3(128), 0, s, x, pe, nw, d.N, d.Q, d.r,
                     d.interaction);
}

void launch_det_value(const Dims& d, const float* F, const float* x, const float* jastrow, const float* norm,
                      float* logpsi, int nw, hipStream_t s, const McmcEpi& epi) {
  const int per = (2 * d.N * d.M + 2 * d.N * d.N + 2 * d.N + 2 * d.K + 2 + 4 + 6 * d.N + 2 + 3 + 1) & ~3;
  auto go = [&](auto kern) {
    hipLaunchKernelGGL(kern, dim3(nw), dim3(64), (size_t)per * sizeof(float), s, F, d.ld_orb, x, jastrow, norm,
                       logpsi, d.N, d.n_up, d.M, d.K, nw, per, epi);
  };
  const int mgv = (d.M + 64 / d.N - 1) / (64 / d.N);
  if (mgv <= 2 && d.N * d.N <= 64) {
    hipLaunchKernelGGL((det_value_kernel<0, true>), dim3((nw + 1) / 2), dim3(64), (size_t)2 * per * sizeof(float), s, F,
                       d.ld_orb, x, jastrow, norm, logpsi, d.N, d.n_up, d.M, d.K, nw, per, epi);
  } else if (mgv <= 2)
    go(det_value_kernel<0>);
  else if (mgv <= 4)
    go(det_value_kernel<4>);
  else if (mgv <= 8)
    go(det_value_kernel<8>);
  else if (mgv <= 16)
    go(det_value_kernel<16>);
  else if (mgv <= 24)
    go(det_value_kernel<24>);
  else if (mgv <= 32)
    go(det_value_kernel<32>);
  else
    go(det_value_kernel<64>);
}

void launch_det_bwd(const Dims& d, const float* F, const float* x, const float* jastrow, const float* norm,
                    const float* ct, float* dF, float* jg, int nw, hipStream_t s) {
  const size_t bytes =
      (size_t)(2 * d.N * d.M + 4 * d.N * d.N + 2 * d.N + 4 * d.K + 2 + 4 + 6 * d.N + 2) * sizeof(float);
  ensure_smem(det_bwd_kernel, bytes);
  hipLaunchKernelGGL(det_bwd_kernel, dim3(nw), dim3(64), bytes, s, F, d.ld_orb, x, jastrow, norm, ct, dF, jg, d.N,
                     d.n_up, d.M, d.K, d.orb_cols);
}

bool det_precontract(const Dims& d) {
  const bool fits = 2 * d.K * d.N <= d.D && d.N <= 32 && d.M <= 16 * 4 * (64 / d.N) && d.M <= 128;
  return fits && !(det_staged(d.N, d.M, d.K) && 2 * d.M * d.N * d.K * d.N <= 8 * 256);
}

static int det_wave_nv(const Dims& d, bool& vec) {
  if (d.N > kDetWaveMaxN || !det_staged(d.N, d.M, d.K)) return 0;
  const int RW = 2 * d.M * d.N * d.K;
  vec = (RW % 4 == 0) && (d.ld_orb % 4 == 0);
  const int units = vec ? d.N * RW / 4 : d.N * RW;
  const int need = (units + 63) / 64;
  for (int v : (vec ? std::initializer_list<int>{1, 2, 3, 5, 8, 12} : std::initializer_list<int>{1, 2, 4, 8, 16}))
    if (need <= v) return v;
  return 0;
}

void launch_det_energy(const Dims& d, const float* F, const float* x, const float* geo, const float* jastrow,
                       const float* norm, float* e_l, float* obs, int nw, hipStream_t s, float* phic) {
  bool vec = false;
  const int nv = phic ? 0 : det_wave_nv(d, vec);
  if (nv > 0) {
    const size_t bytes = (size_t)det_wave_layout(d.N, d.M, d.K).total * sizeof(float);
    auto go = [&](auto kern) {
      ensure_smem(kern, bytes);
      hipLaunchKernelGGL(kern, dim3(nw), dim3(64), bytes, s, F, d.ld_orb, x, geo, jastrow, norm, e_l, obs, d.N, d.n_up,
                         d.M, d.K, d.Q, d.r, d.lambda, d.interaction);
    };
    if (vec) {
      switch (nv) {
        case 1: go(det_energy_wave_kernel<1, true>); break;
        case 2: go(det_energy_wave_kernel<2, true>); break;
        case 3: go(det_energy_wave_kernel<3, true>); break;
        case 5: go(det_energy_wave_kernel<5, true>); break;
        case 8: go(det_energy_wave_kernel<8, true>); break;
        default: go(det_energy_wave_kernel<12, true>); break;
      }
    } else {
      switch (nv) {
        case 1: go(det_energy_wave_kernel<1, false>); break;
        case 2: go(det_energy_wave_kernel<2, false>); break;
        case 4: go(det_energy_wave_kernel<4, false>); break;
        case 8: go(det_energy_wave_kernel<8, false>); break;
        default: go(det_energy_wave_kernel<16, false>); break;
      }
    }
    return;
  }
  const DetSmem L = det_layout(d.N, d.M, d.K, 4, phic != nullptr);
  const size_t bytes = (size_t)L.total * sizeof(float);
  auto go = [&](auto kern) {
    ensure_smem(kern, bytes);
    hipLaunchKernelGGL(kern, dim3(nw), dim3(256), bytes, s, F, d.ld_orb, x, geo, jastrow, norm, e_l, obs, d.N, d.n_up,
                       d.M, d.K, d.Q, d.r, d.lambda, d.interaction, (const float*)phic);
  };
  const int nrw = 2 * d.M * d.N * d.K * d.N;
  if (phic) {
// ... 335 lines not shown
```

### deephall_amd/csrc/dh_internal.h

```cpp
#pragma once
#include <algorithm>
#include <hip/hip_runtime.h>
#include <stdint.h>
#include <stddef.h>

#include "../../include/deephall_amd.h"

namespace dh {

struct Dims {
  int N, n_up, n_dn;
  int T;
  int C;
  int M;
  float Q, r;
  int H, dh, D, L, K;
  int NB;
  int orb_cols;
  int ld_orb;
  int interaction;
  float lambda;
  int sparse;
};
constexpr int kSparseFeatures = 8;
constexpr int kMqkStride = 32;

struct LayerParams {
  const float *Wqkv, *bqkv, *Wol, *bol, *ln1, *Wm, *bm, *ln2;
  const uint16_t *WqkvB, *WolB, *WmB;
  const float *WqkvBT, *WolBT, *WmBT;
  const float *WqkvT, *WolT, *WmT;
  const uint16_t *WqkvP, *WolP, *WmP;
};
struct Params {
  const float* W0;
  LayerParams layer[16];
  const float *Worb, *borb, *jastrow;
  const float* W0qkv;
  const float* WorbT;
  const uint16_t* WorbP;
  const uint16_t* WorbB;
  const float* WorbBT;
  const float* Mqk;
  const float* UT;
  const uint16_t* UP;
  const uint16_t *L1VP, *L1BP;
  const float* L1VT;
  const float* W2T;
  const uint16_t* W2P;
};
inline int ofeat_k(const Dims& d) { return (8 * d.H + 31) / 32 * 32; }

struct Pass {
  int nw;
  int C;
  int rows;
  int rows_pad;
};

enum GemmFamily : int { GEMM_F32_NN = 0, GEMM_F32_NT = 1, GEMM_X6 = 2 };
enum LayerForm : int {
  LF_SEPARATE = 0,
  LF_LN_EPILOGUE,
  LF_CHAIN,
  LF_CHAIN_ATTN,
  LF_LNCH_PAIR,
  LF_LNCH_WHOLE,
  LF_L1CH,
};
enum OrbitalMap : int { ORB_NONE = 0, ORB_GEMM = 1, ORB_IN_CHAIN = 2 };
enum DetStage : int { DET_VALUE = 0, DET_DIRECT = 1, DET_PRECONTRACT = 2, DET_ENV_FIRST = 3 };
struct TrunkRoute {
  int family;
  int input_h;
  int input_qkv;
  int input_skip;
  int form0, form1;
  int attn_feat;
  int h0_epilogue;
  int ofeat;
  int qkv_gemm;
  int orbital;
  int det;
};
constexpr int kTrunkRouteFields = 12;
static_assert(sizeof(TrunkRoute) == kTrunkRouteFields * sizeof(int), "dh_debug_route copies the fields as ints");
int gemm_family(const Dims& d, bool want_x6);
TrunkRoute trunk_route(const Dims& d, int gemm_mode, int C, int rows);

constexpr int kRowPad = 256;
constexpr int kWalkerRowPad = 768;
inline int round_up(int a, int b) { return (a + b - 1) / b * b; }

template <typename Kern>
inline void ensure_smem(Kern kernel, size_t bytes) {
  if (bytes > 65536)
    (void)hipFuncSetAttribute(reinterpret_cast<const void*>(kernel), hipFuncAttributeMaxDynamicSharedMemorySize,
                              (int)bytes);
}

void launch_gemm(const float* X, int ldx, const float* W, int ldw, const float* bias, const float* R, int ldr,
                 float* Y, int ldy, int rows, int ncols, int K, int C, hipStream_t s);
bool launch_gemm_variant(int v, const float* X, int ldx, const float* W, int ldw, const float* bias, const float* R,
                         int ldr, float* Y, int ldy, int rows, int ncols, int K, int C, hipStream_t s);
bool launch_gemm_nt_variant(int v, const float* X, int ldx, const float* Wt, int ldw, const float* bias,
                            const float* R, int ldr, float* Y, int ldy, int rows, int ncols, int K, int C,
                            hipStream_t s);
void launch_gemm_nt(const float* X, int ldx, const float* Wt, int ldw, const float* bias, const float* R, int ldr,
                    float* Y, int ldy, int rows, int ncols, int K, int C, hipStream_t s);
bool gemm_ln_supported(int D, int K);
void launch_gemm_ln(const float* X, int ldx, const float* Wt, int ldw, const float* bias, const float* ln, float* h,
                    int rows, int K, int mode, int bm, hipStream_t s);
int x6_plane_rows(int ncols);
void launch_split_planes(const float* Wt, int ldw, int ncols, int K, uint16_t* Wp, hipStream_t s);
bool gemm_x6_supported(int K);
enum X6Form : int {
  X6D_128x192 = 44,
  X6D_256x128 = 46,
  X6Q_256x128 = 52,
  X6Q_256x256 = 56,
  X6Q_256x192 = 57,
  X6Q_256x160 = 58,
  X6M_256x256 = 76,
  X6M_256x192 = 77,
};
int gemm_x6_choose(int rows, int ncols);
bool launch_gemm_x6_variant(int v, const float* X, int ldx, const uint16_t* Wp, int ldp, const float* bias,
                            const float* R, int ldr, float* Y, int ldy, int rows, int ncols, int K, int C,
                            hipStream_t s);
void launch_gemm_x6(const float* X, int ldx, const uint16_t* Wp, int ldp, const float* bias, const float* R, int ldr,
                    float* Y, int ldy, int rows, int ncols, int K, int C, hipStream_t s);
struct X6Feat {
  const float* W0 = nullptr;
  const float* geo = nullptr;
  int N = 1, n_up = 0;
  const float* W0qkv = nullptr;
  const float* bqkv = nullptr;
  const float* Mqk = nullptr;
  const uint16_t* L1V = nullptr;
  const uint16_t* L1B = nullptr;
};
bool launch_gemm_x6_ln(const float* X, int ldx, const uint16_t* Wp, int ldp, const float* bias, const float* ln,
                       float* h, int rows, int K, int mode, int nw, hipStream_t s, X6Feat feat = X6Feat{});
bool gemm_lnch_supported(int N, int D);
int set_lnch_form(int f);
void launch_gemm_lnch(int N, const float* X, const uint16_t* Wp, int ldp, const float* bias, const float* ln,
                      const float* geo, float* h, int ne, int mode, hipStream_t s,
                      const float* W0f = nullptr, int n_up = 0, int K = 256, const uint16_t* Wv = nullptr,
                      const uint16_t* Wb = nullptr);
void launch_l1_basis(const Dims& d, const float* W0, const float* UT, const float* bol, const float* ln1,
                     const float* Wm, const float* bm, float* BT, float* VT, hipStream_t s);
bool chain_attn_supported(int N, int H, int dh);
void launch_chain_x6(const float* X1, const uint16_t* Wp1, int ldp1, const float* b1, const float* ln1,
                     const uint16_t* Wp2, int ldp2, const float* b2, const float* ln2, const uint16_t* Wp3, int ldp3,
                     const float* b3, int n3, float* Y3, int ldy3, float* h, int rows, X6Feat feat, hipStream_t s,
                     bool store_h = true);
void launch_transpose(const float* src, int ld_src, int rows, int cols, float* dst, int ld_dst, hipStream_t s);

void launch_input(const Dims& d, const float* x, const float* W0, const float* W0qkv, const float* bqkv, float* h,
                  float* qkv, float* geo, int nw, int C, hipStream_t s);
void launch_propose(const Dims& d, const float* x, float* x2, int nw, float width, uint64_t seed, uint64_t step,
                    int64_t walker_offset, const float* noise, int noise_stride, hipStream_t s, float* geo = nullptr);
void launch_accept_propose(const Dims& d, float* x, float* x2, float* geo, float* lp, const float* logpsi2,
                           int32_t* n_acc, int nw, float width, uint64_t seed, uint64_t step, int64_t walker_offset,
                           const float* noise, const float* noise2, hipStream_t s);
void launch_init_walkers(const Dims& d, float* x, int nw, uint64_t seed, int64_t walker_offset, hipStream_t s);

bool attention_takes_features(const Dims& d, int C);
bool attention_mfma_supported(const Dims& d);
void launch_attention_mfma(const Dims& d, const float* qkv, const float* geo, float* o, int nw, hipStream_t s,
                           const float* W0qkv, const float* bqkv);
void launch_attention(const Dims& d, const float* qkv, const float* geo, float* o, int nw, int C, hipStream_t s,
                      const float* W0qkv = nullptr, const float* bqkv = nullptr, const float* Mqk = nullptr);
void launch_lowrank_qk(const Dims& d, const float* W0qkv, const float* bqkv, float* Mqk, hipStream_t s);
void launch_ofeat_weight(const Dims& d, const float* W0qkv, const float* bqkv, const float* Wol, float* UT,
                         hipStream_t s);

void launch_layernorm(const Dims& d, const float* X, const float* Z, const float* ln, const float* geo, float* h,
                      int nw, int C, int mode, hipStream_t s,
                      const float* W0f = nullptr);
bool layer1_ch_supported(const Dims& d);
void launch_layer1_ch(const Dims& d, const float* O, const float* UT, const float* VT, const float* W0f,
                      const float* bol, const float* ln1, const float* ln2, const float* geo, float* h, int nw,
                      hipStream_t s);

struct McmcEpi {
  int on = 0, propose = 0;
  float* x = nullptr;
  float* x2 = nullptr;
  float* geo = nullptr;
  float* lp = nullptr;
  int32_t* nacc = nullptr;
  float width = 0.f;
  uint64_t seed = 0, step = 0;
  int64_t woff = 0;
  const float* noise = nullptr;
  const float* noise2 = nullptr;
};
void launch_det_value(const Dims& d, const float* F, const float* x, const float* jastrow, const float* norm,
                      float* logpsi, int nw, hipStream_t s, const McmcEpi& epi = McmcEpi{});
void launch_histograms(const float* x, int B, int N, int db, int pb, float* dens, float* pair, hipStream_t s);
void launch_monopole_orbitals(const float* pts, int n, int flux, float* out, hipStream_t s);
bool det_precontract(const Dims& d);
void launch_det_energy(const Dims& d, const float* F, const float* x, const float* geo, const float* jastrow,
                       const float* norm, float* e_l, float* obs, int nw, hipStream_t s, float* phic);
size_t det_energy_smem_bytes(const Dims& d);
bool env_first(const Dims& d);
int env_first_k(const Dims& d);
void launch_env_w2(const Dims& d, const float* Worb, float* W2T, hipStream_t s);
void launch_env_first(const Dims& d, const float* h, const float* geo, const float* x, const float* norm,
                      const float* WorbT, const float* borb, const uint16_t* WorbP, const float* W2T,
                      const uint16_t* W2P, bool x6, int nw, float* S, float* FS, float* E2, float* Weff, float* phic,
                      hipStream_t s);
void launch_det_energy_pc(const Dims& d, const float* x, const float* geo, const float* jastrow, const float* norm,
                          float* e_l, float* obs, int nw, hipStream_t s, const float* phic);
void launch_env_leaf_probe(const float* thph, int n, int M, int sq, float* out, hipStream_t s);
void launch_potential(const Dims& d, const float* x, float* pe, int nw, hipStream_t s);
void launch_accept(const Dims& d, float* x, const float* x2, float* lp, const float* logpsi2, int32_t* n_acc,
                   int nw, uint64_t seed, uint64_t step, int64_t walker_offset, const float* noise,
                   int noise_stride, hipStream_t s);
void launch_lp_from_logpsi(const float* logpsi, float* lp, int32_t* n_acc, int nw, hipStream_t s);

size_t kinetic_assembly_lds_bytes(int N);
void launch_kinetic_assembly(const double* x, const double* g, const double* H, int nw, int N, double Q, double r,
                             float* ke, float* mom, hipStream_t s);

void launch_stats(const float* e_l, const float* obs, const int32_t* n_acc, int B, int steps, int penalties,
                  float* out, hipStream_t s);
void launch_loss_diff(const float* e_l, const float* obs, int B, const float* g, float lz_penalty, float lz_center,
                      float l2_penalty, float* diff, float* nvalid, hipStream_t s);

constexpr int kGradChunk = 512;
constexpr int kLnRowsPerBlock = 64;
int grad_chunks(int rows);
int ln_bwd_blocks(int rows);
void launch_ln_fwd(const float* a, const float* z, const float* ln, float* out, int rows, int D, hipStream_t s);
void launch_ln_bwd(const float* a, const float* z, const float* ln, const float* dy, const float* dres, float* da,
                   float* dz, float* pg, int rows, int D, hipStream_t s);
void launch_ln_bwd_rows(const float* a, const float* z, const float* ln, const float* dy, const float* dres,
                        float* da, float* dz, float* pg, int rows, int D, int rpb, hipStream_t s);
void launch_attn_bwd(const Dims& d, const float* qkv, const float* dO, float* dqkv, int nw, hipStream_t s);
void launch_tn_partial(const float* X, int ldx, const float* Y, int ldy, int rows, int M, int Nc, float* P,
                       hipStream_t s);
void launch_colsum_partial(const float* Y, int ldy, int rows, int Nc, float* P, hipStream_t s);
void launch_w0_partial(const Dims& d, const float* geo, const float* Y, int ldy, int rows, float* P, hipStream_t s);
void launch_reduce2d(const float* P, int nchunk, size_t stride, int ldp, int nr, int nc, float* out, int ldo,
                     float scale, int acc, hipStream_t s);
void launch_small_gemm(int M, int N, int K, const float* A, int lda, int ta, const float* B, int ldb, int tb, float* C,
                       int ldc, int acc, hipStream_t s);
void launch_copy2d(const float* src, int lds, float* dst, int ldd, int nr, int nc, hipStream_t s);
void launch_cotangent(const float* diff, const float* nvalid, int B, int part, float* ct, hipStream_t s);
void launch_adam(float* p, const float* g, float* mu, float* nu, size_t n, float lr, float b1, float b2, float eps,
                 int step, hipStream_t s);
void launch_sparse_fold(const float* W8, const float* b8, const float* Wl, const float* bl, int real_part, int D,
                        int NK, int M, float* Wfull, int ldw, float* bfull, hipStream_t s);
void launch_sparse_unfold(const float* dWfull, int ldw, const float* dbfull, const float* Wl, int D, int NK, int M,
                          float* dW8, float* db8, int acc, hipStream_t s);
struct SparseBlocks {
  const float* W8[4];
  const float* b8[4];
  int n;
};
void launch_sparse_lll_grad(SparseBlocks blk, const float* dWfull, int ldw, const float* dbfull, int D, int NK, int M,
                            float* dWl, float* dbl, int acc, hipStream_t s);

size_t laughlin_smem_bytes(int N);
void launch_laughlin(const Dims& d, const float* x, const int* expo, float* logpsi, float* e_l, float* obs, int nw,
                     hipStream_t s);

size_t cf_smem_bytes(int N, int n_dense, bool energy);
void launch_cf(const Dims& d, const float* x, const int* tab, int n_dense, float* logpsi, float* e_l, float* obs,
               int nw, hipStream_t s);

size_t pfaffian_smem_bytes(int N, bool energy);
void launch_pfaffian(const Dims& d, const float* x, int p, float* logpsi, float* e_l, float* obs, int nw,
                     hipStream_t s);

void launch_det_bwd(const Dims& d, const float* F, const float* x, const float* jastrow, const float* norm,
                    const float* ct, float* dF, float* jg, int nw, hipStream_t s);

struct KfacSlot {
  int n;
  size_t off;
// ... 74 lines not shown
```

### deephall_amd/csrc/gemm_x6.hip

```cpp
#include <cstdlib>
#include <type_traits>

#include "attn_val.h"
#include "dh_internal.h"
#include "device_common.h"

#ifndef CHAIN_STAMP
#define CHAIN_STAMP 0
#endif

namespace dh {

#if CHAIN_STAMP
constexpr int CHAIN_STAMP_WG = 512, CHAIN_NSTAMP = 16;
__device__ unsigned long long g_chain_stamp[2 * CHAIN_STAMP_WG * CHAIN_NSTAMP];
#define CHAIN_T(i)                                                                                  \
  do {                                                                                              \
    if (threadIdx.x == 0 && blockIdx.x < CHAIN_STAMP_WG)                                            \
      g_chain_stamp[((NA > 0) * CHAIN_STAMP_WG + blockIdx.x) * CHAIN_NSTAMP + (i)] = __builtin_amdgcn_s_memtime(); \
  } while (0)
extern "C" int dh_debug_chain_stamps(unsigned long long* out, int n) {
  n = n < 2 * CHAIN_STAMP_WG * CHAIN_NSTAMP ? n : 2 * CHAIN_STAMP_WG * CHAIN_NSTAMP;
  return hipMemcpyFromSymbol(out, HIP_SYMBOL(g_chain_stamp), n * sizeof(unsigned long long)) == hipSuccess ? 0 : -1;
}
#else
#define CHAIN_T(i)
#endif

typedef float f32x16 __attribute__((ext_vector_type(16)));
typedef float f32x4 __attribute__((ext_vector_type(4)));
typedef __bf16 bf16x8 __attribute__((ext_vector_type(8)));

namespace {

constexpr int X6_BK = 32;

int cu_count_x6() {
  static int n = 0;
  if (n == 0) {
    int dev = 0;
    (void)hipGetDevice(&dev);
    if (hipDeviceGetAttribute(&n, hipDeviceAttributeMultiprocessorCount, dev) != hipSuccess || n <= 0) n = 256;
  }
  return n;
}

typedef float f32x2 __attribute__((ext_vector_type(2)));
typedef __bf16 bf16x2 __attribute__((ext_vector_type(2)));
typedef uint32_t u32x4v __attribute__((ext_vector_type(4)));

__device__ __forceinline__ uint32_t pk_bf16(float x, float y) {
  return __builtin_bit_cast(uint32_t, __builtin_convertvector((f32x2){x, y}, bf16x2));
}
__device__ __forceinline__ float lo_f(uint32_t u) { return __uint_as_float(u << 16); }
__device__ __forceinline__ float hi_f(uint32_t u) { return __uint_as_float(u & 0xffff0000u); }

__device__ __forceinline__ void split3(const float4& u, const float4& v, bf16x8& h, bf16x8& m, bf16x8& l) {
  const float a[8] = {u.x, u.y, u.z, u.w, v.x, v.y, v.z, v.w};
  u32x4v H, Mv, Lv;
#pragma unroll
  for (int p = 0; p < 4; ++p) {
    const float x = a[2 * p], y = a[2 * p + 1];
    const uint32_t h2 = pk_bf16(x, y);
    const float rx = x - lo_f(h2), ry = y - hi_f(h2);
    const uint32_t m2 = pk_bf16(rx, ry);
    const float sx = rx - lo_f(m2), sy = ry - hi_f(m2);
    H[p] = h2;
    Mv[p] = m2;
    Lv[p] = pk_bf16(sx, sy);
  }
  h = __builtin_bit_cast(bf16x8, H);
  m = __builtin_bit_cast(bf16x8, Mv);
  l = __builtin_bit_cast(bf16x8, Lv);
}

template <int TN, int B_PLANE>
__device__ __forceinline__ void ktile_pipelined(const char* Bs, const char* Bn, f32x16 (&acc)[TN], bf16x8 (&nb)[3],
                                                const bf16x8& c0, const bf16x8& c1, const bf16x8& c2,
                                                const float4& u, const float4& v, bf16x8& n0, bf16x8& n1,
                                                bf16x8& n2) {
  bf16x8 fb[2][3];
  auto ld = [&](const char* base, int j, bf16x8(&d)[3]) __attribute__((always_inline)) {
    d[0] = *reinterpret_cast<const bf16x8*>(base + j * 1024);
    d[1] = *reinterpret_cast<const bf16x8*>(base + B_PLANE + j * 1024);
    d[2] = *reinterpret_cast<const bf16x8*>(base + 2 * B_PLANE + j * 1024);
  };
  fb[0][0] = nb[0];
  fb[0][1] = nb[1];
// ... 854 lines not shown
          }
          *reinterpret_cast<f32x4*>(Y + (size_t)(rw0 + rb * 16 + l16) * ldy + n) = c;
        }
      }
#pragma unroll
      for (int rb = 0; rb < 4; ++rb)
#pragma unroll
        for (int cb = 0; cb < TNC; ++cb) acc[rb][cb] = (f32x4){0.f, 0.f, 0.f, 0.f};
      stored = true;
    } else {
      asm volatile("s_waitcnt vmcnt(0)" ::: "memory");
#pragma unroll
      for (int cb = 0; cb < TNC; ++cb) {
#pragma unroll
        for (int rb = 0; rb < 4; ++rb) {
          const int r = rw0 + rb * 16 + l16, n = cw0 + cb * 16 + 4 * kg;
          const f32x4 c = acc[rb][cb];
          acc[rb][cb] = (f32x4){0.f, 0.f, 0.f, 0.f};
          if (r >= rows) continue;
#pragma unroll
          for (int e = 0; e < 4; ++e) {
            if (n + e >= ncols) continue;
            float x = c[e];
            if (bfl[rb] != 0.f) x += bias[n + e];
            if (HAS_R) x += R[(size_t)r * ldr + n + e];
            Y[(size_t)r * ldy + n + e] = x;
          }
        }
      }
      asm volatile("s_waitcnt vmcnt(0)" ::: "memory");
    }
  }
}

template <int TNC, bool DMA4 = false>
void launch_x6m_t(const float* X, int ldx, const uint16_t* Wp, int ldp, const float* bias, const float* R, int ldr,
                  float* Y, int ldy, int rows, int ncols, int K, int C, hipStream_t s) {
  constexpr int BM = 256, BN = 32 * TNC;
  const int ntm = (rows + BM - 1) / BM, ntn = (ncols + BN - 1) / BN;
  const size_t smem = 2ull * (BM * 32 * 4 + 3 * BN * 32 * 2);
  int grid = std::min(ntm * ntn, cu_count_x6());
  grid = std::max(8, grid / 8 * 8);
  if (R) {
    ensure_smem(gemm_x6m_kernel<TNC, true, DMA4>, smem);
    hipLaunchKernelGGL((gemm_x6m_kernel<TNC, true, DMA4>), dim3(grid), dim3(512), smem, s, X, ldx, Wp, ldp, bias, R,
                       ldr, Y, ldy, rows, ncols, K, C, ntm, ntn);
  } else {
    ensure_smem(gemm_x6m_kernel<TNC, false, DMA4>, smem);
    hipLaunchKernelGGL((gemm_x6m_kernel<TNC, false, DMA4>), dim3(grid), dim3(512), smem, s, X, ldx, Wp, ldp, bias,
                       R, ldr, Y, ldy, rows, ncols, K, C, ntm, ntn);
  }
}

__global__ void split_planes_kernel(const float* __restrict__ Wt, int ldw, int ncols, int K, int ldp, uint16_t* Wp) {
  const size_t i = (size_t)blockIdx.x * blockDim.x + threadIdx.x;
  const size_t plane = (size_t)ldp * K;
  if (i >= plane) return;
  const int n = (int)(i / K), k = (int)(i % K);
  const float a = n < ncols ? Wt[(size_t)n * ldw + k] : 0.f;
  const __bf16 a0 = (__bf16)a;
  const float r1 = a - (float)a0;
  const __bf16 a1 = (__bf16)r1;
  const __bf16 a2 = (__bf16)(r1 - (float)a1);
  Wp[i] = __builtin_bit_cast(uint16_t, a0);
  Wp[plane + i] = __builtin_bit_cast(uint16_t, a1);
  Wp[2 * plane + i] = __builtin_bit_cast(uint16_t, a2);
}


constexpr int CH_BM = 96, CH_BN = 256, CH_K = 256;
constexpr int CH_KO = 32;

struct ChainArgs {
  const float* X1;
  const uint16_t *Wp1, *Wp2, *Wp3;
  int ldp1, ldp2, ldp3;
  const float *b1, *ln1, *b2, *ln2, *b3;
  int n3, ldy3;
  float* Y3;
  float* h;
  int rows;
  X6Feat feat;
  int store_h;
};

constexpr int CS_NW = 8, CS_RB = CH_BM / 32, CS_PD = 4, CS_LSP = 264;
constexpr int CS_PRMF = 5 * 256;
constexpr size_t CS_PLANE = (size_t)CH_BM * CS_LSP * 2, CS_SMEM = 3 * CS_PLANE + 2 * CS_NW * CH_BM * 4 + CS_PRMF * 4;
static_assert(CS_SMEM <= 163840, "chain LDS");

__device__ __forceinline__ void split4(const float4& x, uint2& h, uint2& m, uint2& l) {
  const float a[4] = {x.x, x.y, x.z, x.w};
  uint32_t H[2], Mv[2], Lv[2];
#pragma unroll
  for (int p = 0; p < 2; ++p) {
    const float u = a[2 * p], v = a[2 * p + 1];
    const uint32_t h2 = pk_bf16(u, v);
    const float ru = u - lo_f(h2), rv = v - hi_f(h2);
    const uint32_t m2 = pk_bf16(ru, rv);
    H[p] = h2;
    Mv[p] = m2;
    Lv[p] = pk_bf16(ru - lo_f(m2), rv - hi_f(m2));
  }
  h = make_uint2(H[0], H[1]);
  m = make_uint2(Mv[0], Mv[1]);
  l = make_uint2(Lv[0], Lv[1]);
}

template <int NA = 0>
__global__ __launch_bounds__(512) void chain_x6s_kernel(ChainArgs a) {
  constexpr int RB = CS_RB, PD = CS_PD, LSP = CS_LSP;
  using K16 = std::integral_constant<int, CH_K / 16>;
  using KP1 = std::integral_constant<int, (NA > 0 ? CH_KO / 16 : CH_K / 16)>;
  using K2 = std::integral_constant<int, 2>;
  extern __shared__ float4 smem4[];
  char* smem = reinterpret_cast<char*>(smem4);
  float* part = reinterpret_cast<float*>(smem + 3 * CS_PLANE);
  float* prm = part + 2 * CS_NW * CH_BM;
  const int tid = threadIdx.x, lane = tid & 63;
  const int wid = __builtin_amdgcn_readfirstlane(tid >> 6);
  const int l32 = lane & 31, lh = lane >> 5;
  int bid = blockIdx.x;
  {
    const int nblk = gridDim.x, q = nblk / 8, r8 = nblk % 8, xcd = bid % 8, slot = bid / 8;
    bid = (xcd < r8 ? xcd * (q + 1) : r8 * (q + 1) + (xcd - r8) * q) + slot;
  }
  constexpr int TRW = NA > 0 ? (CH_BM / NA) * NA : CH_BM;
  const int row0 = bid * TRW, rows = min(a.rows, row0 + TRW);
  auto lbar = []() __attribute__((always_inline)) {
    asm volatile("s_waitcnt lgkmcnt(0)" ::: "memory");
    __builtin_amdgcn_s_barrier();
    asm volatile("" ::: "memory");
  };
  CHAIN_T(0);
  for (int q = tid; q < CS_PRMF; q += 512)
    prm[q] = q < 512 ? a.ln1[q] : (q < 768 ? a.b2[q - 512] : a.ln2[q - 768]);
  auto pl = [&](int p, int r, int c) __attribute__((always_inline)) {
    return smem + (size_t)p * CS_PLANE + (size_t)r * (LSP * 2) + c * 2;
  };
  auto put4 = [&](int r, int c, const float4& x) __attribute__((always_inline)) {
    uint2 h, m, l;
    split4(x, h, m, l);
    *reinterpret_cast<uint2*>(pl(0, r, c)) = h;
    *reinterpret_cast<uint2*>(pl(1, r, c)) = m;
    *reinterpret_cast<uint2*>(pl(2, r, c)) = l;
  };
  auto get4 = [&](int r, int c) __attribute__((always_inline)) {
    const uint2 h = *reinterpret_cast<const uint2*>(pl(0, r, c));
    const uint2 m = *reinterpret_cast<const uint2*>(pl(1, r, c));
    const uint2 l = *reinterpret_cast<const uint2*>(pl(2, r, c));
    return make_float4((lo_f(h.x) + lo_f(m.x)) + lo_f(l.x), (hi_f(h.x) + hi_f(m.x)) + hi_f(l.x),
                       (lo_f(h.y) + lo_f(m.y)) + lo_f(l.y), (hi_f(h.y) + hi_f(m.y)) + hi_f(l.y));
  };

  f32x16 acc[RB];
  bf16x8 bq[PD][3];
  const uint16_t* wr = nullptr;
  size_t plane = 0;
  auto prefetch = [&](const uint16_t* Wp, int ldp, int col0, auto nkt_) __attribute__((always_inline)) {
    constexpr int NKT = decltype(nkt_)::value, KK = 16 * NKT;
    plane = (size_t)ldp * KK;
    wr = Wp + (size_t)(col0 + 32 * wid + l32) * KK + 8 * lh;
#pragma unroll
    for (int d = 0; d < (PD < NKT ? PD : NKT); ++d)
#pragma unroll
      for (int p = 0; p < 3; ++p) bq[d][p] = *reinterpret_cast<const bf16x8*>(wr + p * plane + 16 * d);
  };
  auto gemm = [&](auto tr_, auto nkt_, auto accumulate_) __attribute__((always_inline)) {
    constexpr bool TR = decltype(tr_)::value;
    constexpr int nk = decltype(nkt_)::value;
    auto mf = [](const bf16x8& w, const bf16x8& x, const f32x16& c) __attribute__((always_inline)) {
      if constexpr (TR)
        return __builtin_amdgcn_mfma_f32_32x32x16_bf16(x, w, c, 0, 0, 0);
      else
        return __builtin_amdgcn_mfma_f32_32x32x16_bf16(w, x, c, 0, 0, 0);
    };
    if constexpr (!decltype(accumulate_)::value) {
#pragma unroll
      for (int rb = 0; rb < RB; ++rb)
#pragma unroll
        for (int e = 0; e < 16; ++e) acc[rb][e] = 0.f;
    }
    bf16x8 ca[RB][3];
    auto lda = [&](int kt, bf16x8(&d)[RB][3]) __attribute__((always_inline)) {
#pragma unroll
      for (int rb = 0; rb < RB; ++rb)
#pragma unroll
        for (int p = 0; p < 3; ++p)
          d[rb][p] = *reinterpret_cast<const bf16x8*>(pl(p, 32 * rb + l32, 16 * kt + 8 * lh));
    };
    lda(0, ca);
#pragma unroll
    for (int kt = 0; kt < nk; ++kt) {
// ... 300 lines not shown
      } else if (j < 24) {
        const int c = 8 * ((j - 4) / 5) + (j - 4) % 5;
        const uint32_t h = *reinterpret_cast<const uint16_t*>(pl(0, r, c));
        const uint32_t m = *reinterpret_cast<const uint16_t*>(pl(1, r, c));
        const uint32_t l = *reinterpret_cast<const uint16_t*>(pl(2, r, c));
        z = (lo_f(h) + lo_f(m)) + lo_f(l);
      } else if (j == 24) {
        z = 1.f;
      } else if (j == 25) {
        z = -st.x;
      }
      rv[p] = j == 26 ? 1.f : st.y * z;
    }
    lbar();
#pragma unroll
    for (int p = 0; p < RP; ++p) {
      const int r = (tid >> 5) + 16 * p;
      const float v = rv[p];
      const uint32_t h2 = pk_bf16(v, 0.f);
      const float rx = v - lo_f(h2);
      const uint32_t m2 = pk_bf16(rx, 0.f);
      const uint32_t l2 = pk_bf16(rx - lo_f(m2), 0.f);
      *reinterpret_cast<uint16_t*>(pl(0, r, j)) = (uint16_t)h2;
      *reinterpret_cast<uint16_t*>(pl(1, r, j)) = (uint16_t)m2;
      *reinterpret_cast<uint16_t*>(pl(2, r, j)) = (uint16_t)l2;
    }
    lbar();
    CHAIN_T(4);
    CHAIN_T(5);
    gemm(NoTr{}, K2{}, Zero{});
    prefetch(a.feat.L1B, a.ldp2, 0, K2{});
#pragma unroll
    for (int rb = 0; rb < RB; ++rb)
#pragma unroll
      for (int e = 0; e < 16; ++e) acc[rb][e] = tanh_rat(acc[rb][e]);
    gemm(NoTr{}, K2{}, Accum{});
    CHAIN_T(6);
    if (a.Wp3 && 32 * wid < a.n3) prefetch(a.Wp3, a.ldp3, 0, K16{});
#pragma unroll
    for (int rb = 0; rb < RB; ++rb)
#pragma unroll
      for (int e = 0; e < 16; ++e) x[rb][e] = acc[rb][e];
  } else {
  layernorm(prm);
  CHAIN_T(4);
#pragma unroll
  for (int rb = 0; rb < RB; ++rb)
#pragma unroll
    for (int g = 0; g < 4; ++g)
      put4(32 * rb + l32, colof(g), make_float4(x[rb][4 * g], x[rb][4 * g + 1], x[rb][4 * g + 2], x[rb][4 * g + 3]));
  lbar();
  CHAIN_T(5);
  gemm(NoTr{}, K16{}, Zero{});
  CHAIN_T(6);
  if (a.Wp3 && 32 * wid < a.n3) prefetch(a.Wp3, a.ldp3, 0, K16{});
#pragma unroll
  for (int rb = 0; rb < RB; ++rb)
#pragma unroll
    for (int g = 0; g < 4; ++g) {
      const float4 bv = *reinterpret_cast<const float4*>(prm + 512 + colof(g));
      const float4 h1 = get4(32 * rb + l32, colof(g));
      x[rb][4 * g] = h1.x + tanh_rat(acc[rb][4 * g] + bv.x);
      x[rb][4 * g + 1] = h1.y + tanh_rat(acc[rb][4 * g + 1] + bv.y);
      x[rb][4 * g + 2] = h1.z + tanh_rat(acc[rb][4 * g + 2] + bv.z);
      x[rb][4 * g + 3] = h1.w + tanh_rat(acc[rb][4 * g + 3] + bv.w);
    }
  }
  CHAIN_T(7);
  layernorm(prm + 768);
  CHAIN_T(8);
#pragma unroll
  for (int rb = 0; rb < RB; ++rb) {
    const int r = row0 + 32 * rb + l32;
#pragma unroll
    for (int g = 0; g < 4; ++g) {
      const float4 y = make_float4(x[rb][4 * g], x[rb][4 * g + 1], x[rb][4 * g + 2], x[rb][4 * g + 3]);
      if (a.Wp3) put4(32 * rb + l32, colof(g), y);
      if (a.store_h && r < rows) *reinterpret_cast<float4*>(a.h + (size_t)r * CH_BN + colof(g)) = y;
    }
  }
  if (!a.Wp3) return;
  lbar();
  CHAIN_T(9);
  for (int col0 = 0; col0 < a.n3; col0 += CH_BN) {
    if (col0 + 32 * wid >= a.n3) continue;
    gemm(Tr{}, K16{}, Zero{});
    if (col0 < 3 * CH_BN) CHAIN_T(10 + 2 * (col0 / CH_BN));
    const int c = col0 + 32 * wid + l32;
    const bool cok = c < a.n3;
    const float bv = cok ? a.b3[c] : 0.f;
    if (col0 + CH_BN + 32 * wid < a.n3) prefetch(a.Wp3, a.ldp3, col0 + CH_BN, K16{});
    const int nrow = min(CH_BM, rows - row0), ldb = a.ldy3 * 4;
    const auto rs = __builtin_amdgcn_make_buffer_rsrc(a.Y3 + (size_t)row0 * a.ldy3, (short)0, nrow * ldb, 0x00020000);
    const int vo = cok ? 4 * lh * ldb + 4 * c : 0x7fffffff;
    if (nrow == CH_BM) {
#pragma unroll
      for (int rb = 0; rb < RB; ++rb) {
#pragma unroll
        for (int q = 0; q < 16; ++q)
          __builtin_amdgcn_raw_buffer_store_b32(__builtin_bit_cast(uint32_t, acc[rb][q] + bv), rs, vo,
                                                (32 * rb + (q & 3) + 8 * (q >> 2)) * ldb, 0);
      }
    } else {
#pragma unroll
      for (int rb = 0; rb < RB; ++rb) {
#pragma unroll
        for (int q = 0; q < 16; ++q) {
          const int r = 32 * rb + (q & 3) + 8 * (q >> 2) + 4 * lh;
          const int v = (cok && r < nrow) ? 4 * c + r * ldb : 0x7fffffff;
          __builtin_amdgcn_raw_buffer_store_b32(__builtin_bit_cast(uint32_t, acc[rb][q] + bv), rs, v, 0, 0);
        }
      }
    }
    if (col0 < 3 * CH_BN) CHAIN_T(11 + 2 * (col0 / CH_BN));
  }
}


}

int x6_plane_rows(int ncols) { return round_up(ncols, kRowPad) + kRowPad; }

void launch_split_planes(const float* Wt, int ldw, int ncols, int K, uint16_t* Wp, hipStream_t s) {
  const int ldp = x6_plane_rows(ncols);
  const size_t n = (size_t)ldp * K;
  hipLaunchKernelGGL(split_planes_kernel, dim3((unsigned)((n + 255) / 256)), dim3(256), 0, s, Wt, ldw, ncols, K, ldp,
                     Wp);
}

bool gemm_x6_supported(int K) { return K % X6_BK == 0; }

namespace {
using X6Launch = void (*)(const float* X, int ldx, const uint16_t* Wp, int ldp, const float* bias, const float* R,
                          int ldr, float* Y, int ldy, int rows, int ncols, int K, int C, hipStream_t s);
template <int TN, int NW, int ST, int WN = 1>
void launch_x6d_plain(const float* X, int ldx, const uint16_t* Wp, int ldp, const float* bias, const float* R, int ldr,
                      float* Y, int ldy, int rows, int ncols, int K, int C, hipStream_t s) {
  launch_x6d_t<TN, NW, ST, 0, WN>(X, ldx, Wp, ldp, bias, R, ldr, Y, ldy, rows, ncols, K, C, s);
}
void launch_x6d_grid96(const float* X, int ldx, const uint16_t* Wp, int ldp, const float* bias, const float* R, int ldr,
                       float* Y, int ldy, int rows, int ncols, int K, int C, hipStream_t s) {
  if (round_up(rows, 96) <= round_up(rows, 256))
    launch_x6d_plain<2, 3, 3, 4>(X, ldx, Wp, ldp, bias, R, ldr, Y, ldy, rows, ncols, K, C, s);
  else
    launch_x6d_plain<2, 2, 3, 4>(X, ldx, Wp, ldp, bias, R, ldr, Y, ldy, rows, ncols, K, C, s);
}
const struct {
  int code;
  X6Launch launch;
} kX6Forms[] = {
    {X6D_128x192, launch_x6d_plain<6, 4, 2>},
    {X6D_256x128, launch_x6d_plain<4, 8, 2>},
    {43, launch_x6d_plain<8, 4, 2>},
    {45, launch_x6d_plain<4, 4, 2>},
    {40, launch_x6d_plain<8, 8, 3>},
    {41, launch_x6d_plain<6, 8, 3>},
    {60, launch_x6d_grid96},
    {61, launch_x6d_plain<2, 2, 3, 4>},
    {62, launch_x6d_plain<2, 4, 3, 4>},
    {50, launch_x6q_t<8>},
    {51, launch_x6q_t<6>},
    {X6Q_256x128, launch_x6q_t<4>},
    {X6Q_256x256, launch_x6q_t<8, true>},
    {X6Q_256x192, launch_x6q_t<6, true>},
    {X6Q_256x160, launch_x6q_t<5, true>},
    {80, launch_x6m_t<8>},
    {81, launch_x6m_t<6>},
    {82, launch_x6m_t<5>},
    {83, launch_x6m_t<4>},
    {X6M_256x256, launch_x6m_t<8, true>},
    {X6M_256x192, launch_x6m_t<6, true>},
    {79, launch_x6m_t<4, true>},
    {90, launch_x6m_t<5, true>},
};
}

bool launch_gemm_x6_variant(int v, const float* X, int ldx, const uint16_t* Wp, int ldp, const float* bias,
                            const float* R, int ldr, float* Y, int ldy, int rows, int ncols, int K, int C,
                            hipStream_t s) {
  for (const auto& f : kX6Forms)
    if (f.code == v) {
      f.launch(X, ldx, Wp, ldp, bias, R, ldr, Y, ldy, rows, ncols, K, C, s);
      return true;
    }
  return false;
}

int gemm_x6_choose(int rows, int ncols) {
  int v;
  if (rows >= 65536 && ncols % 256 == 0 && ncols >= 512) {
    v = X6M_256x256;
  } else if (rows >= 65536 && ncols == 192) {
    v = X6M_256x192;
  } else if (rows >= 65536) {
    v = X6Q_256x256;
    if (ncols < 1024) {
      const int tns[4] = {8, 6, 5, 4}, vs[4] = {X6Q_256x256, X6Q_256x192, X6Q_256x160, X6Q_256x128};
      int best = round_up(ncols, 256);
      for (int q = 1; q < 4; ++q) {
        const int padded = round_up(ncols, 32 * tns[q]);
        if (padded < best) {
          best = padded;
          v = vs[q];
        }
      }
    }
  } else {
    v = (ncols % 192 == 0) ? X6D_128x192 : X6D_256x128;
  }
  return v;
}

void launch_gemm_x6(const float* X, int ldx, const uint16_t* Wp, int ldp, const float* bias, const float* R, int ldr,
                    float* Y, int ldy, int rows, int ncols, int K, int C, hipStream_t s) {
  launch_gemm_x6_variant(gemm_x6_choose(rows, ncols), X, ldx, Wp, ldp, bias, R, ldr, Y, ldy, rows, ncols, K, C, s);
}

bool launch_gemm_x6_ln(const float* X, int ldx, const uint16_t* Wp, int ldp, const float* bias, const float* ln,
                       float* h, int rows, int K, int mode, int nw, hipStream_t s, X6Feat feat) {
  if (mode != 0) feat = X6Feat{};
  if (nw == 0) {
    const int cus = cu_count_x6();
    const int bm[3] = {96, 128, 64}, cost[3] = {280, 305, 230}, form[3] = {1, 8, 2};
    long best = -1;
    for (int q = 0; q < 3; ++q) {
      const long t = (long)(((rows + bm[q] - 1) / bm[q] + cus - 1) / cus) * cost[q];
      if (best < 0 || t < best) {
        best = t;
        nw = form[q];
      }
    }
  }
#define DH_X6LN(TNV, NWV, WNV)                                                                               \
  do {                                                                                                       \
    if (mode == 0)                                                                                           \
      launch_x6d_t<TNV, NWV, 3, 1, WNV>(X, ldx, Wp, ldp, bias, h, 256, h, 256, rows, 256, K, 1, s, ln, feat); \
    else                                                                                                     \
      launch_x6d_t<TNV, NWV, 3, 2, WNV>(X, ldx, Wp, ldp, bias, h, 256, h, 256, rows, 256, K, 1, s, ln);      \
  } while (0)
  switch (nw) {
    case 1: DH_X6LN(2, 3, 4); break;
    case 2: DH_X6LN(2, 2, 4); break;
    case 3: DH_X6LN(8, 3, 1); break;
    case 4: DH_X6LN(8, 4, 1); break;
    case 8: DH_X6LN(2, 4, 4); break;
    default: return false;
  }
#undef DH_X6LN
  return true;
}

void launch_chain_x6(const float* X1, const uint16_t* Wp1, int ldp1, const float* b1, const float* ln1,
                     const uint16_t* Wp2, int ldp2, const float* b2, const float* ln2, const uint16_t* Wp3, int ldp3,
                     const float* b3, int n3, float* Y3, int ldy3, float* h, int rows, X6Feat feat, hipStream_t s,
                     bool store_h) {
  ChainArgs a{X1, Wp1, Wp2, Wp3, ldp1, ldp2, ldp3, b1, ln1, b2, ln2, b3, n3, ldy3, Y3, h, rows, feat, store_h ? 1 : 0};
  auto k = chain_x6s_kernel<0>;
  if (feat.W0qkv) {
    switch (feat.N) {
      case 2: k = chain_x6s_kernel<2>; break;
      case 3: k = chain_x6s_kernel<3>; break;
      case 4: k = chain_x6s_kernel<4>; break;
      case 6: k = chain_x6s_kernel<6>; break;
      case 8: k = chain_x6s_kernel<8>; break;
      case 10: k = chain_x6s_kernel<10>; break;
      default: k = chain_x6s_kernel<20>; break;
    }
  }
  const int trw = feat.W0qkv ? (CH_BM / feat.N) * feat.N : CH_BM;
  ensure_smem(k, CS_SMEM);
  hipLaunchKernelGGL(k, dim3((rows + trw - 1) / trw), dim3(512), CS_SMEM, s, a);
}

bool chain_attn_supported(int N, int H, int dh) {
  return H == 4 && dh == 64 && (N == 2 || N == 3 || N == 4 || N == 6 || N == 8 || N == 10 || N == 20);
}

}
```

### deephall_amd/csrc/trunk_route.cpp

```cpp
#include "dh_internal.h"

namespace dh {

int gemm_family(const Dims& d, bool want_x6) {
  const bool nt = d.D % 32 == 0;
  return nt && want_x6 && gemm_x6_supported(d.D) ? GEMM_X6 : nt ? GEMM_F32_NT : GEMM_F32_NN;
}

TrunkRoute trunk_route(const Dims& d, int gemm_mode, int C, int rows) {
  const int D = d.D;
  const bool channels = C > 1;
  const bool unfused = gemm_mode == DH_GEMM_X6_ALL_UNFUSED;
  TrunkRoute r{};
  r.family = gemm_family(d, channels ? gemm_mode != DH_GEMM_F32 : (gemm_mode == DH_GEMM_X6_ALL || unfused));
  const bool x6 = r.family == GEMM_X6, nt = r.family != GEMM_F32_NN;
  const bool fused = d.L > 0 && attention_takes_features(d, C);
  r.attn_feat = fused;
  r.input_qkv = d.L > 0 && !fused;
  r.qkv_gemm = 1;
  r.form0 = r.form1 = LF_SEPARATE;
  r.det = !channels ? DET_VALUE : env_first(d) ? DET_ENV_FIRST : det_precontract(d) ? DET_PRECONTRACT : DET_DIRECT;
  r.orbital = r.det == DET_ENV_FIRST ? ORB_NONE : ORB_GEMM;

  if (!channels && nt && gemm_ln_supported(D, D)) {
    r.form0 = r.form1 = LF_LN_EPILOGUE;
    r.h0_epilogue = fused && x6;
    if (d.L > 0 && x6 && D == 256 && (rows < 65536 || d.N >= 20)) {
      r.form0 = fused && chain_attn_supported(d.N, d.H, d.dh) ? LF_CHAIN_ATTN : LF_CHAIN;
      r.form1 = LF_CHAIN;
      r.ofeat = r.form0 == LF_CHAIN_ATTN;
      r.qkv_gemm = 0;
      r.orbital = ORB_IN_CHAIN;
    }
  } else if (channels) {
    r.ofeat = fused;
    if (x6 && C == 2 * d.N + 5 && !unfused && gemm_lnch_supported(d.N, D)) {
      r.form0 = fused && d.H == 4 ? LF_LNCH_WHOLE : LF_LNCH_PAIR;
      r.form1 = LF_LNCH_PAIR;
      r.h0_epilogue = fused;
    } else if (fused && D == 256 && (d.N == 10 || d.N == 20)) {
      r.h0_epilogue = 1;
      if (d.dh == 64 && d.H == 4 && layer1_ch_supported(d) && !unfused) r.form0 = LF_L1CH;
    }
  }
  r.input_h = !r.h0_epilogue;
  r.input_skip = !channels && r.h0_epilogue;
  return r;
}

}
```

### include/deephall_amd.h

```cpp
#ifndef DEEPHALL_AMD_H
#define DEEPHALL_AMD_H

#include <stddef.h>
#include <stdint.h>

#ifdef __cplusplus
extern "C" {
#endif

#define DH_OK 0
#define DH_EINVAL -1
#define DH_EHIP -2
#define DH_ENOMEM -3
#define DH_ESTATE -4

#define DH_INTERACTION_COULOMB 0
#define DH_INTERACTION_HARMONIC 1
#define DH_NETWORK_PSIFORMER 0
#define DH_NETWORK_LAUGHLIN 1
#define DH_NETWORK_JAIN 2
#define DH_NETWORK_PFAFFIAN 3
#define DH_ORBITAL_FULL 0
#define DH_ORBITAL_SPARSE 1

// ... 66 lines not shown
int dh_set_gemm_mode(dh_handle* h, int mode);

size_t dh_workspace_bytes(const dh_handle* h, int batch, int op);

int dh_logpsi(dh_handle* h, const float* x, int B, float* logpsi, void* ws, size_t ws_bytes, void* stream);

int dh_mcmc_step(dh_handle* h, float* x, float* lp, int32_t* n_accept, int B, int steps, float width,
                 uint64_t seed, uint64_t counter, int64_t walker_offset, const float* noise, void* ws,
                 size_t ws_bytes, void* stream);

int dh_local_energy(dh_handle* h, const float* x, int B, float* e_l, float* obs, void* ws, size_t ws_bytes,
                    void* stream);

#define DH_NSTATS 16
#define DH_STAT_ENERGY_RE 0
#define DH_STAT_ENERGY_IM 1
#define DH_STAT_CLIPPED_RE 2
#define DH_STAT_CLIPPED_IM 3
#define DH_STAT_ERE2 4
#define DH_STAT_KINETIC_RE 5
#define DH_STAT_KINETIC_IM 6
#define DH_STAT_POTENTIAL 7
#define DH_STAT_LZ 8
#define DH_STAT_LZ2 9
#define DH_STAT_L2 10
#define DH_STAT_PMOVE 11
#define DH_STAT_NVALID 12
#define DH_STAT_CLIPPED_LZ2 13
#define DH_STAT_CLIPPED_LZ 14
#define DH_STAT_CLIPPED_L2 15
int dh_energy_stats(dh_handle* h, const float* e_l, const float* obs, const int32_t* n_accept, int B, int steps,
                    int penalties, float* out, void* stream);

int dh_loss_diff(dh_handle* h, const float* e_l, const float* obs, int B, const float* stats, float lz_penalty,
                 float lz_center, float l2_penalty, float* diff, float* nvalid, void* stream);

#define DH_NFID 5
#define DH_FID_M 0
#define DH_FID_S_RE 1
#define DH_FID_S_IM 2
#define DH_FID_S2 3
#define DH_FID_N 4
int dh_fidelity_partial(const float* logpsi, const float* logphi, int B, double* part, void* stream);
int dh_fidelity_residual(const float* logpsi, const float* logphi, int B, const double* total, float* resid,
                         void* stream);

int dh_potential(dh_handle* h, const float* x, int B, float* pe, void* stream);

int dh_histograms(const float* x, int B, int nelec, int density_bins, int pair_bins, float* density, float* pair,
                  void* stream);
int dh_monopole_orbitals(const float* points, int n, int flux, float* out, void* stream);

int dh_mh_init(const float* logpsi, float* lp, int32_t* n_accept, int B, void* stream);
int dh_mh_propose(const float* x, float* x2, int B, int nelec, float width, uint64_t seed, uint64_t step,
                  int64_t walker_offset, const float* noise, void* stream);
int dh_mh_accept(float* x, const float* x2, float* lp, const float* logpsi2, int32_t* n_accept, int B, int nelec,
                 uint64_t seed, uint64_t step, int64_t walker_offset, const float* noise, void* stream);
int dh_kinetic_from_derivatives(const double* x, const double* grad, const double* hess, int B, int nelec, double Q,
                                double r, float* ke, float* mom, void* stream);

int dh_profile_enable(dh_handle* h, int on);
int dh_profile_read(dh_handle* h, double* out, int reset);

int dh_debug_trunk(dh_handle* h, const float* x, int B, int op, void* ws, size_t ws_bytes, void* stream);
size_t dh_debug_f_offset(const dh_handle* h, int B, int op);
int dh_debug_env_leaf(const float* thph, int n, int M, int sq, float* out, void* stream);
int dh_debug_gemm(int variant, const float* X, int ldx, const float* W, int ldw, const float* bias, const float* R,
                  int ldr, float* Y, int ldy, int rows, int ncols, int K, int C, void* stream);

int dh_debug_gemm_ln(int mode, int bm, const float* X, int ldx, const float* Wt, int ldw, const float* bias,
                     const float* ln, float* h, int rows, int K, void* stream);

int dh_debug_gemm_x6_ln(int mode, int nw, const float* X, int ldx, const uint16_t* Wp, int ldp, const float* bias,
                        const float* ln, float* h, int rows, int K, void* stream);
int dh_debug_chain_x6(const float* X1, const uint16_t* Wp1, int ldp1, const float* b1, const float* ln1,
                      const uint16_t* Wp2, int ldp2, const float* b2, const float* ln2, const uint16_t* Wp3,
                      int ldp3, const float* b3, int n3, float* Y3, int ldy3, float* h, int rows, void* stream);

int dh_debug_gemm_lnch(int N, int mode, const float* X, const uint16_t* Wp, int ldp, const float* bias,
                       const float* ln, const float* geo, float* h, int ne, void* stream);

int dh_debug_gemm_x6_choice(int rows, int ncols);
int dh_debug_route(const dh_handle* h, int B, int op, int* out, int n);
int dh_debug_x6_plane_rows(int ncols);
int dh_debug_split_planes(const float* Wt, int ldw, int ncols, int K, uint16_t* Wp, void* stream);
int dh_debug_gemm_x6(int variant, const float* X, int ldx, const uint16_t* Wp, int ldp, const float* bias,
                     const float* R, int ldr, float* Y, int ldy, int rows, int ncols, int K, int C, void* stream);

int dh_init_walkers(dh_handle* h, float* x, int B, uint64_t seed, int64_t walker_offset, void* stream);

#ifdef __cplusplus
}
#endif
#endif
```

Before: 807,600 local-energies/s.

## Fuse determinant value evaluation into the chained trunk GEMM kernel tail

Adds a determinant-tail variant of the chained x6 trunk kernel. The final orbital GEMM output is staged in LDS, and the half-wave determinant/logpsi body runs on those tile rows inside the same kernel. This avoids writing F to global memory and launching a separate det_value kernel during MCMC value passes. The cost is more LDS pressure and register use in the chain kernel, and only the orbital GEMM columns handled per wave are computed, in a single pass.

Result: faster. 822,900 local-energies/s, median of 6 (+1.9%).

```diff
diff --git a/deephall_amd/_lib.py b/deephall_amd/_lib.py
--- a/deephall_amd/_lib.py
+++ b/deephall_amd/_lib.py
@@ -62,6 +62,8 @@
     "dh_debug_gemm_x6",
     "dh_debug_gemm_x6_choice",
     "dh_debug_route",
+    "dh_debug_set_det_in_chain",
+    "dh_debug_det_in_chain",
     "dh_ref_layout",
     "dh_set_params_ref",
     "dh_vjp_workspace_bytes",
@@ -199,6 +201,10 @@
     lib.dh_debug_gemm_x6_choice.restype = i32
     lib.dh_debug_route.argtypes = [vp, i32, i32, C.POINTER(i32), i32]
     lib.dh_debug_route.restype = i32
+    lib.dh_debug_set_det_in_chain.argtypes = [i32]
+    lib.dh_debug_set_det_in_chain.restype = i32
+    lib.dh_debug_det_in_chain.argtypes = [vp, i32, i32]
+    lib.dh_debug_det_in_chain.restype = i32
     lib.dh_ref_layout.argtypes = [vp, C.POINTER(sz), i32]
     lib.dh_ref_layout.restype = i32
     lib.dh_set_params_ref.argtypes = [vp, vp, sz, vp]
diff --git a/deephall_amd/csrc/api.cpp b/deephall_amd/csrc/api.cpp
--- a/deephall_amd/csrc/api.cpp
+++ b/deephall_amd/csrc/api.cpp
@@ -767,6 +767,8 @@
   const int nw, C, rows;
   const TrunkRoute r;
   const bool keep_h;
+  const ChainDet* det = nullptr;
+  const bool keep_F = false;
   const int D = d.D, KO = ofeat_k(d);
   const int ch = C > 1 ? PK_CH : 0;
   const double R = rows, DD = D, f4 = 4.0;
@@ -794,7 +796,8 @@
     launch_chain_x6(w.o, attn ? P.UP : lp.WolP, x6_plane_rows(D), lp.bol, lp.ln1, lp.WmP, x6_plane_rows(D), lp.bm,
                     lp.ln2, last ? P.WorbP : P.layer[l + 1].WqkvP, x6_plane_rows(n3),
                     last ? P.borb : P.layer[l + 1].bqkv, n3, last ? w.F : w.qkv, last ? d.ld_orb : 3 * D, w.h, rows,
-                    feat, s, !last || keep_h);
+                    feat, s, !last || keep_h,
+                    last ? det : nullptr, !(last && det) || keep_F);
   }
   void layer_ln_epilogue(int l) const {
     const LayerParams& lp = P.layer[l];
@@ -886,8 +889,26 @@
 };
 
 int run_trunk(dh_handle* h, const float* x, int nw, int C, const Work& w, hipStream_t s, bool geo_ready = false,
-              bool keep_h = false) {
-  return Trunk{h, h->d, h->p, w, s, nw, C, nw * h->d.N * C, w.route, keep_h}.run(x, geo_ready);
+              bool keep_h = false, const ChainDet* det = nullptr, bool keep_F = false) {
+  return Trunk{h, h->d, h->p, w, s, nw, C, nw * h->d.N * C, w.route, keep_h, det, keep_F}.run(x, geo_ready);
+}
+
+ChainDet chain_det(const dh_handle* h, const float* x, int nw, float* logpsi, const McmcEpi& epi) {
+  const Dims& d = h->d;
+  ChainDet c;
+  c.x = x;
+  c.jastrow = h->p.jastrow;
+  c.norm = h->norm;
+  c.logpsi = logpsi;
+  c.N = d.N;
+  c.n_up = d.n_up;
+  c.M = d.M;
+  c.K = d.K;
+  c.nw = nw;
+  c.per = det_value_per(d);
+  c.ldf = det_chain_ldf(d);
+  c.epi = epi;
+  return c;
 }
 
 int launch_trial(dh_handle* h, const float* x, float* logpsi, float* e_l, float* obs, int nw, hipStream_t s) {
@@ -908,6 +929,10 @@
 int value_pass(dh_handle* h, const float* x, int nw, const Work& w, float* logpsi, hipStream_t s,
                bool geo_ready = false, const McmcEpi& epi = McmcEpi{}) {
   if (h->analytic()) return launch_trial(h, x, logpsi, nullptr, nullptr, nw, s);
+  if (w.route.det_in_chain && !h->prof.on) {
+    const ChainDet det = chain_det(h, x, nw, logpsi, epi);
+    return run_trunk(h, x, nw, 1, w, s, geo_ready, false, &det);
+  }
   if (int rc = run_trunk(h, x, nw, 1, w, s, geo_ready)) return rc;
   {
     PROF(PK_DET_VALUE, 0.0, 4.0 * nw * h->d.N * h->d.ld_orb);
@@ -1859,6 +1884,10 @@
   if (!w.F)
     return fail(DH_EINVAL, "dh_debug_trunk: this config's local energy goes envelope first and maps no orbital "
                            "features F over the channel rows");
+  if (op != 1 && w.route.det_in_chain) {
+    const ChainDet det = chain_det(h, x, B, w.logpsi, McmcEpi{});
+    return run_trunk(h, x, B, 1, w, (hipStream_t)stream, false, true, &det, true);
+  }
   return run_trunk(h, x, B, op == 1 ? h->d.C : 1, w, (hipStream_t)stream, false, true);
 }
 
@@ -1948,6 +1977,14 @@
 }
 
 int dh_debug_set_lnch_form(int form) { return set_lnch_form(form); }
+
+int dh_debug_set_det_in_chain(int on) { return set_det_in_chain(on); }
+
+int dh_debug_det_in_chain(const dh_handle* h, int B, int op) {
+  if (!h || h->analytic() || B < 1) return fail(DH_EINVAL, "bad route query");
+  const int C = op == 1 ? h->d.C : 1;
+  return trunk_route(h->d, h->gemm_mode, C, B * h->d.N * C).det_in_chain;
+}
 
 int dh_debug_gemm_ln(int mode, int bm, const float* X, int ldx, const float* Wt, int ldw, const float* bias,
                      const float* ln, float* h, int rows, int K, void* stream) {
diff --git a/deephall_amd/csrc/det.hip b/deephall_amd/csrc/det.hip
--- a/deephall_amd/csrc/det.hip
+++ b/deephall_amd/csrc/det.hip
@@ -5,9 +5,6 @@
 #include "device_common.h"
 #include "mcmc_common.h"
 
-#ifndef DET_LU_REG
-#define DET_LU_REG 0
-#endif
 #ifndef DET_WAVE_SQ
 #define DET_WAVE_SQ 1
 #endif
@@ -36,16 +33,10 @@
 #define DET_T(slot, i)
 #endif
 
+#include "det_value.h"
+
 namespace dh {
 namespace {
-
-__device__ inline float ipow(float b, int e) { return e < 0 ? 0.f : (e == 0 ? 1.f : powf(b, (float)e)); }
-__device__ inline float ipow_sq(float b, int e) {
-  float r = 1.f;
-  for (; e > 0; e >>= 1, b *= b)
-    if (e & 1) r *= b;
-  return r;
-}
 
 struct FView {
   const float* F;
@@ -57,41 +48,6 @@
     return cf{F[base + (size_t)(blk * 2) * MNK + off], F[base + (size_t)(blk * 2 + 1) * MNK + off]};
   }
 };
-
-struct EnvLeaf {
-  cf e0, dth, dph, lb, d2th;
-};
-__device__ __forceinline__ float env_gauge(float ct, int M) {
-  return (float)(M - 1) * __builtin_rintf(64.f * ct) * (1.f / 128.f);
-}
-__device__ inline EnvLeaf env_leaf(float th, float ph, int p, int M, float norm, bool leaves, float gauge = 0.f,
-                                   bool sq = false) {
-  const int a = p, b = M - 1 - p;
-  const float m = 0.5f * (float)(a - b) - gauge;
-  float c, s;
-  sincosf(0.5f * th, &s, &c);
-  float sph, cph;
-  sincosf(m * ph, &sph, &cph);
-  const float R = sq ? ipow_sq(c, a) * ipow_sq(s, b) : ipow(c, a) * ipow(s, b);
-  EnvLeaf L;
-  L.e0 = cf{norm * R * cph, norm * R * sph};
-  if (leaves) {
-    const float fa = (float)a, fb = (float)b;
-    auto pw = [sq](float x, int e) { return sq ? (e < 0 ? 0.f : ipow_sq(x, e)) : ipow(x, e); };
-    const float R1 = 0.5f * (fb * pw(c, a + 1) * pw(s, b - 1) - fa * pw(c, a - 1) * pw(s, b + 1));
-    const float R2 = 0.25f * (fb * (fb - 1.f) * pw(c, a + 2) * pw(s, b - 2) - fb * (fa + 1.f) * R -
-                              fa * (fb + 1.f) * R + fa * (fa - 1.f) * pw(c, a - 2) * pw(s, b + 2));
-    float st, ct;
-    sincosf(th, &st, &ct);
-    L.dth = cf{norm * R1 * cph, norm * R1 * sph};
-    L.d2th = cf{norm * R2 * cph, norm * R2 * sph};
-    L.dph = cf{-m * L.e0.im / st, m * L.e0.re / st};
-    const float cot = ct / st;
-    const float k2 = m * m / (st * st);
-    L.lb = cf{L.d2th.re - k2 * L.e0.re + cot * L.dth.re, L.d2th.im - k2 * L.e0.im + cot * L.dth.im};
-  }
-  return L;
-}
 
 __device__ inline cf env_flow2(const cf& e0, const cf& dth, const cf& d2th, float m, float st, float ct, float sp,
                                float cp, int k) {
@@ -114,78 +70,6 @@
   return r;
 }
 
-__device__ inline void find_pivot(const cf* A, int lda, int N, int p, int* piv, int tid, int width) {
-  if (tid < width) {
-    const int lane = tid;
-    float best = -1.f;
-    int bi = N;
-    for (int r = p + lane; r < N; r += width) {
-      const float v = cabs1(A[r * lda + p]);
-      if (v > best) {
-        best = v;
-        bi = r;
-      }
-    }
-    for (int o = width >> 1; o > 0; o >>= 1) {
-      const float ob = __shfl_xor(best, o, width);
-      const int oi = __shfl_xor(bi, o, width);
-      if (ob > best || (ob == best && oi < bi)) {
-        best = ob;
-        bi = oi;
-      }
-    }
-    if (lane == 0) *piv = (bi < N) ? bi : p;
-  }
-}
-
-__device__ __forceinline__ void eliminate(cf* A, int lda, int N, int ncol, bool gj, cf* fac, int* piv, cf* logdet,
-                          int tid = threadIdx.x, int nt = blockDim.x, int width = 64) {
-  if (tid == 0) *logdet = cf{0.f, 0.f};
-  __syncthreads();
-  for (int p = 0; p < N; ++p) {
-    find_pivot(A, lda, N, p, piv, tid, width);
-    __syncthreads();
-    const int pr = *piv;
-    if (pr != p) {
-      for (int c = tid; c < ncol; c += nt) {
-        const cf t = A[p * lda + c];
-        A[p * lda + c] = A[pr * lda + c];
-        A[pr * lda + c] = t;
-      }
-    }
-    __syncthreads();
-    const cf P = A[p * lda + p];
-    if (tid == 0) {
-      const float mag = sqrtf(P.re * P.re + P.im * P.im);
-      logdet->re += logf(mag);
-      logdet->im += atan2f(P.im, P.re) + (pr != p ? kPi : 0.f);
-    }
-    const cf Pinv = cdiv(cf{1.f, 0.f}, P);
-    __syncthreads();
-    if (gj) {
-      for (int r = tid; r < N; r += nt) fac[r] = (r == p) ? cf{0.f, 0.f} : A[r * lda + p];
-      for (int c = tid; c < ncol; c += nt) A[p * lda + c] = A[p * lda + c] * Pinv;
-    } else {
-      for (int r = tid; r < N; r += nt) fac[r] = (r > p) ? A[r * lda + p] * Pinv : cf{0.f, 0.f};
-    }
-    __syncthreads();
-    const int r0 = gj ? 0 : p + 1;
-    const int c0 = gj ? 0 : p;
-    const int nr = N - r0, nc = ncol - c0;
-    for (int idx = tid; idx < nr * nc; idx += nt) {
-      const int r = r0 + idx / nc, c = c0 + idx % nc;
-      if (r == p) continue;
-      const cf f = fac[r];
-      cf v = A[r * lda + c];
-      const cf a = A[p * lda + c];
-      v.re -= f.re * a.re - f.im * a.im;
-      v.im -= f.re * a.im + f.im * a.re;
-      A[r * lda + c] = v;
-    }
-    __syncthreads();
-  }
-}
-
 template <int NMAX>
 __device__ __forceinline__ cf gj_inverse_cols(cf (&col)[NMAX], int N) {
   auto is = [](int r, int q) __attribute__((always_inline)) {
@@ -244,243 +128,16 @@
   return cf{lre, lim};
 }
 
-template <int NMAX>
-__device__ __forceinline__ cf lu_logdet_cols(cf (&col)[NMAX], int N, int lane, int width) {
-  auto is = [](int r, int q) __attribute__((always_inline)) {
-    int m = r == q;
-    asm volatile("" : "+v"(m));
-    return m != 0;
-  };
-  auto pick = [&](int q) __attribute__((always_inline)) {
-    cf v = col[0];
-#pragma unroll
-    for (int r = 1; r < NMAX; ++r)
-      if (is(r, q)) v = col[r];
-    return v;
-  };
-  float lre = 0.f, lim = 0.f;
-  for (int p = 0; p < N; ++p) {
-    float best = -1.f;
-    int bi = N;
-#pragma unroll
-    for (int r = 0; r < NMAX; ++r) {
-      if (r >= p && r < N) {
-        const float v = cabs1(col[r]);
-        if (v > best) {
-          best = v;
-          bi = r;
-        }
-      }
-    }
-    int pr = __shfl(bi, p, width);
-    pr = pr < N ? pr : p;
-    if (pr != p) {
-      const cf a = pick(p), b = pick(pr);
-#pragma unroll
-      for (int r = 0; r < NMAX; ++r) {
-        if (is(r, p)) col[r] = b;
-        if (is(r, pr)) col[r] = a;
-      }
-    }
-    const cf mine = pick(p);
-    const cf P{__shfl(mine.re, p, width), __shfl(mine.im, p, width)};
-    const float mag = sqrtf(P.re * P.re + P.im * P.im);
-    lre += logf(mag);
-    lim += atan2f(P.im, P.re) + (pr != p ? kPi : 0.f);
-    const cf Pinv = cdiv(cf{1.f, 0.f}, P);
-#pragma unroll
-    for (int r = 0; r < NMAX; ++r) {
-      if (r > p && r < N) {
-#pragma clang fp contract(off)
-        const cf c = col[r];
-        const cf fl{c.re * Pinv.re - c.im * Pinv.im, __builtin_fmaf(c.im, Pinv.re, c.re * Pinv.im)};
-        const cf f{__shfl(fl.re, p, width), __shfl(fl.im, p, width)};
-        if (lane >= p) {
-          const float tre = __builtin_fmaf(f.re, mine.re, -(f.im * mine.im));
-          const float tim = __builtin_fmaf(f.im, mine.re, f.re * mine.im);
-          col[r] = cf{c.re - tre, c.im - tim};
-        }
-      }
-    }
-  }
-  return cf{lre, lim};
-}
-
-__device__ inline double jastrow_pair(double r, double al, double cst, double* f1, double* f2) {
-  const double ar = al + r;
-  *f1 = (cst * al * al) / (ar * ar);
-  *f2 = -2.0 * (cst * al * al) / (ar * ar * ar);
-  return -(cst * al * al) / ar;
-}
-
 template <int MGV, bool HW = false>
 __global__ __launch_bounds__(64) void det_value_kernel(const float* __restrict__ Fp, int ldF, const float* x,
                                  const float* __restrict__ jas, const float* __restrict__ norm, float* __restrict__ logpsi,
                                  int N, int n_up, int M, int K, int nw, int per, McmcEpi epi) {
-  static_assert(!HW || MGV == 0, "half-wave form: serial contraction only");
   extern __shared__ float sm_all[];
   const int half = HW ? (int)(threadIdx.x >> 5) : 0;
-  float* sm_raw = sm_all + half * per;
-  cf* E0 = reinterpret_cast<cf*>(sm_raw);
-  cf* A = E0 + N * M;
-  cf* fac = A + N * N;
-  cf* ld = fac + N;
-  cf* logdet = ld + K;
-  int* piv = reinterpret_cast<int*>(logdet + 1);
   const int bw = HW ? 2 * (int)blockIdx.x + half : (int)blockIdx.x;
-  const bool live = bw < nw;
-  const int b = live ? bw : nw - 1;
-  const int tid = HW ? (int)(threadIdx.x & 31) : (int)threadIdx.x, nt = HW ? 32 : 64, width = HW ? 32 : 64;
-  double* cart = reinterpret_cast<double*>(piv + 2);
-  DET_T(0, 0);
-  for (int idx = tid; idx < N * M; idx += nt) {
-    const int i = idx / M, p = idx % M;
-    E0[idx] = env_leaf(x[2 * (b * N + i)], x[2 * (b * N + i) + 1], p, M, norm[p], false, 0.f, true).e0;
-  }
-  for (int i = tid; i < N; i += nt) {
-    double st, ct, sp, cp;
-    sincos((double)x[2 * (b * N + i)], &st, &ct);
-    sincos((double)x[2 * (b * N + i) + 1], &sp, &cp);
-    cart[3 * i] = st * cp;
-    cart[3 * i + 1] = st * sp;
-    cart[3 * i + 2] = ct;
-  }
-  __syncthreads();
-  DET_T(0, 1);
-  double Jw = 0.0;
-  {
-    const double ap = jas[0], aa = jas[1];
-    for (int q = tid; q < N * N; q += nt) {
-      const int i = q / N, j = q - (q / N) * N;
-      if (j <= i) continue;
-      const double dx = cart[3 * j] - cart[3 * i], dy = cart[3 * j + 1] - cart[3 * i + 1],
-                   dz = cart[3 * j + 2] - cart[3 * i + 2];
-      const double r = sqrt(dx * dx + dy * dy + dz * dz);
-      const bool same = (i < n_up) == (j < n_up);
-      double f1, f2;
-      Jw += jastrow_pair(r, same ? ap : aa, same ? 0.25 : 0.5, &f1, &f2);
-    }
-    for (int o = width >> 1; o > 0; o >>= 1) Jw += __shfl_xor(Jw, o, width);
-  }
-  DET_T(0, 2);
-  const int G = 64 / N, gj = tid % N, gg = tid / N, NK = N * K, MNK = M * NK;
-  for (int k = 0; k < K; ++k) {
-    if constexpr (MGV == 0) {
-      for (int idx = tid; idx < N * N; idx += nt) {
-        const int i = idx / N, j = idx % N;
-        const int blk = (i >= n_up && n_up > 0) ? 1 : 0;
-        const float* rp = Fp + ((size_t)b * N + i) * ldF + (size_t)blk * 2 * MNK + (size_t)j * K + k;
-        cf acc{0.f, 0.f};
-        for (int p0 = 0; p0 < M; p0 += 16) {
-          float fr[16], fi[16];
-#pragma unroll
-          for (int q = 0; q < 16; ++q) {
-            const size_t p = (size_t)min(p0 + q, M - 1);
-            fr[q] = rp[p * NK];
-            fi[q] = rp[(size_t)MNK + p * NK];
-          }
-#pragma unroll
-          for (int q = 0; q < 16; ++q)
-            if (p0 + q < M) cfma(acc, cf{fr[q], fi[q]}, E0[i * M + p0 + q]);
-        }
-        A[idx] = acc;
-      }
-    }
-    if constexpr (MGV > 0) {
-      constexpr int NF = 2 * (MGV > 0 ? MGV : 1);
-      auto ldrow = [&](int i, float (&f)[NF]) __attribute__((always_inline)) {
-        const int blk = (i >= n_up && n_up > 0) ? 1 : 0;
-        const float* rp = Fp + ((size_t)b * N + i) * ldF + (size_t)blk * 2 * MNK + (size_t)gj * K + k;
-#pragma unroll
-        for (int u = 0; u < MGV; ++u) {
-          const size_t m = (size_t)min(gg + G * u, M - 1);
-          f[2 * u] = rp[m * NK];
-          f[2 * u + 1] = rp[(size_t)MNK + m * NK];
-        }
-      };
-      auto contract = [&](int i, const float (&f)[NF]) __attribute__((always_inline)) {
-        cf acc{0.f, 0.f};
-#pragma unroll
-        for (int u = 0; u < MGV; ++u) {
-          const int m = gg + G * u;
-          const bool ok = gg < G && m < M;
-          cfma(acc, cf{ok ? f[2 * u] : 0.f, ok ? f[2 * u + 1] : 0.f}, E0[i * M + min(m, M - 1)]);
-        }
-        float re = acc.re, im = acc.im;
-        for (int q = 1; q < G; ++q) {
-          re += __shfl(acc.re, gj + N * q, 64);
-          im += __shfl(acc.im, gj + N * q, 64);
-        }
-        if (gg == 0) A[i * N + gj] = cf{re, im};
-      };
-      float fa[NF], fb[NF];
-      if constexpr (MGV <= 24) {
-        ldrow(0, fa);
-        for (int i = 0; i < N; i += 2) {
-          ldrow(min(i + 1, N - 1), fb);
-          contract(i, fa);
-          ldrow(min(i + 2, N - 1), fa);
-          if (i + 1 < N) contract(i + 1, fb);
-        }
-      } else {
-        for (int i = 0; i < N; ++i) {
-          ldrow(i, fa);
-          contract(i, fa);
-        }
-      }
-    }
-    __syncthreads();
-    DET_T(0, 3);
-    if (N <= 8 && DET_LU_REG) {
-      cf col[8];
-#pragma unroll
-      for (int r = 0; r < 8; ++r) col[r] = (r < N && tid < N) ? A[r * N + tid] : cf{0.f, 0.f};
-      const cf l = lu_logdet_cols<8>(col, N, tid, width);
-      if (tid == 0) ld[k] = l;
-    } else {
-      eliminate(A, N, N, N, false, fac, piv, logdet, tid, nt, width);
-      if (tid == 0) ld[k] = *logdet;
-    }
-    __syncthreads();
-    DET_T(0, 4);
-  }
-  float* lpv = reinterpret_cast<float*>(cart + 3 * N);
-  if (tid == 0 && live) {
-    float lmax = -INFINITY;
-    for (int k = 0; k < K; ++k) lmax = fmaxf(lmax, ld[k].re);
-    float zr = 0.f, zi = 0.f;
-    for (int k = 0; k < K; ++k) {
-      const float mag = expf(ld[k].re - lmax);
-      zr += mag * cosf(ld[k].im);
-      zi += mag * sinf(ld[k].im);
-    }
-    float val_re = 0.5f * logf(zr * zr + zi * zi) + lmax;
-    float val_im = atan2f(zi, zr);
-    logpsi[2 * b] = val_re + (float)Jw;
-    logpsi[2 * b + 1] = val_im;
-    *lpv = val_re + (float)Jw;
-  }
-  DET_T(0, 5);
-  if (!epi.on) return;
-  __syncthreads();
-  if (!live || tid >= N) return;
-  const float lp2 = 2.f * *lpv;
-  const bool cond = accept_one(lp2, epi.lp[b], b, N, epi.seed, epi.step, epi.woff, epi.noise);
-  const int e = b * N + tid;
-  float th = epi.x[2 * e], ph = epi.x[2 * e + 1];
-  if (cond) {
-    th = x[2 * e];
-    ph = x[2 * e + 1];
-    epi.x[2 * e] = th;
-    epi.x[2 * e + 1] = ph;
-    if (tid == 0) {
-      epi.lp[b] = lp2;
-      epi.nacc[b] += 1;
-    }
-  }
-  if (epi.propose)
-    propose_one(th, ph, epi.x2, epi.geo, e, b, tid, N, epi.width, epi.seed, epi.step + 1, epi.woff, epi.noise2);
-  DET_T(0, 6);
+  const int tid = HW ? (int)(threadIdx.x & 31) : (int)threadIdx.x;
+  det_value_body<MGV, HW>(sm_all + half * per, FRowsGlobal{Fp, ldF, N}, x, jas, norm, logpsi, N, n_up, M, K, bw, nw,
+                          tid, epi, BlockSync{});
 }
 
 #ifndef ENV_REG
@@ -1990,13 +1647,13 @@
 
 void launch_det_value(const Dims& d, const float* F, const float* x, const float* jastrow, const float* norm,
                       float* logpsi, int nw, hipStream_t s, const McmcEpi& epi) {
-  const int per = (2 * d.N * d.M + 2 * d.N * d.N + 2 * d.N + 2 * d.K + 2 + 4 + 6 * d.N + 2 + 3 + 1) & ~3;
+  const int per = det_value_per(d);
   auto go = [&](auto kern) {
     hipLaunchKernelGGL(kern, dim3(nw), dim3(64), (size_t)per * sizeof(float), s, F, d.ld_orb, x, jastrow, norm,
                        logpsi, d.N, d.n_up, d.M, d.K, nw, per, epi);
   };
   const int mgv = (d.M + 64 / d.N - 1) / (64 / d.N);
-  if (mgv <= 2 && d.N * d.N <= 64) {
+  if (det_value_half_wave(d)) {
     hipLaunchKernelGGL((det_value_kernel<0, true>), dim3((nw + 1) / 2), dim3(64), (size_t)2 * per * sizeof(float), s, F,
                        d.ld_orb, x, jastrow, norm, logpsi, d.N, d.n_up, d.M, d.K, nw, per, epi);
   } else if (mgv <= 2)
diff --git a/deephall_amd/csrc/det_value.h b/deephall_amd/csrc/det_value.h
--- /dev/null
+++ b/deephall_amd/csrc/det_value.h
@@ -0,0 +1,413 @@
+#pragma once
+#include "dh_internal.h"
+#include "device_common.h"
+#include "mcmc_common.h"
+
+#ifndef DET_LU_REG
+#define DET_LU_REG 0
+#endif
+#ifndef DET_T
+#define DET_T(slot, i)
+#endif
+
+namespace dh {
+
+struct BlockSync {
+  __device__ __forceinline__ void operator()() const { __syncthreads(); }
+};
+struct WaveSync {
+  __device__ __forceinline__ void operator()() const {
+    asm volatile("s_waitcnt lgkmcnt(0)" ::: "memory");
+    __builtin_amdgcn_wave_barrier();
+    asm volatile("" ::: "memory");
+  }
+};
+
+struct FRowsGlobal {
+  const float* __restrict__ F;
+  int ld, N;
+  __device__ __forceinline__ const float* operator()(int b, int i) const { return F + ((size_t)b * N + i) * ld; }
+};
+struct FRowsTile {
+  const float* F;
+  int ld, N, b0;
+  __device__ __forceinline__ const float* operator()(int b, int i) const { return F + ((b - b0) * N + i) * ld; }
+};
+
+__device__ inline float ipow(float b, int e) { return e < 0 ? 0.f : (e == 0 ? 1.f : powf(b, (float)e)); }
+__device__ inline float ipow_sq(float b, int e) {
+  float r = 1.f;
+  for (; e > 0; e >>= 1, b *= b)
+    if (e & 1) r *= b;
+  return r;
+}
+
+struct EnvLeaf {
+  cf e0, dth, dph, lb, d2th;
+};
+__device__ __forceinline__ float env_gauge(float ct, int M) {
+  return (float)(M - 1) * __builtin_rintf(64.f * ct) * (1.f / 128.f);
+}
+__device__ inline EnvLeaf env_leaf(float th, float ph, int p, int M, float norm, bool leaves, float gauge = 0.f,
+                                   bool sq = false) {
+  const int a = p, b = M - 1 - p;
+  const float m = 0.5f * (float)(a - b) - gauge;
+  float c, s;
+  sincosf(0.5f * th, &s, &c);
+  float sph, cph;
+  sincosf(m * ph, &sph, &cph);
+  const float R = sq ? ipow_sq(c, a) * ipow_sq(s, b) : ipow(c, a) * ipow(s, b);
+  EnvLeaf L;
+  L.e0 = cf{norm * R * cph, norm * R * sph};
+  if (leaves) {
+    const float fa = (float)a, fb = (float)b;
+    auto pw = [sq](float x, int e) { return sq ? (e < 0 ? 0.f : ipow_sq(x, e)) : ipow(x, e); };
+    const float R1 = 0.5f * (fb * pw(c, a + 1) * pw(s, b - 1) - fa * pw(c, a - 1) * pw(s, b + 1));
+    const float R2 = 0.25f * (fb * (fb - 1.f) * pw(c, a + 2) * pw(s, b - 2) - fb * (fa + 1.f) * R -
+                              fa * (fb + 1.f) * R + fa * (fa - 1.f) * pw(c, a - 2) * pw(s, b + 2));
+    float st, ct;
+    sincosf(th, &st, &ct);
+    L.dth = cf{norm * R1 * cph, norm * R1 * sph};
+    L.d2th = cf{norm * R2 * cph, norm * R2 * sph};
+    L.dph = cf{-m * L.e0.im / st, m * L.e0.re / st};
+    const float cot = ct / st;
+    const float k2 = m * m / (st * st);
+    L.lb = cf{L.d2th.re - k2 * L.e0.re + cot * L.dth.re, L.d2th.im - k2 * L.e0.im + cot * L.dth.im};
+  }
+  return L;
+}
+
+__device__ inline void find_pivot(const cf* A, int lda, int N, int p, int* piv, int tid, int width) {
+  if (tid < width) {
+    const int lane = tid;
+    float best = -1.f;
+    int bi = N;
+    for (int r = p + lane; r < N; r += width) {
+      const float v = cabs1(A[r * lda + p]);
+      if (v > best) {
+        best = v;
+        bi = r;
+      }
+    }
+    for (int o = width >> 1; o > 0; o >>= 1) {
+      const float ob = __shfl_xor(best, o, width);
+      const int oi = __shfl_xor(bi, o, width);
+      if (ob > best || (ob == best && oi < bi)) {
+        best = ob;
+        bi = oi;
+      }
+    }
+    if (lane == 0) *piv = (bi < N) ? bi : p;
+  }
+}
+
+struct PinnedLu {
+  static __device__ __forceinline__ float mag2(cf P) {
+#pragma clang fp contract(off)
+    const float rr = P.re * P.re, ii = P.im * P.im;
+    return rr + ii;
+  }
+  static __device__ __forceinline__ cf factor(cf c, cf Pinv) {
+#pragma clang fp contract(off)
+    const float rr = c.re * Pinv.re, ii = c.im * Pinv.im, ri = c.re * Pinv.im;
+    return cf{rr - ii, __builtin_fmaf(c.im, Pinv.re, ri)};
+  }
+  static __device__ __forceinline__ cf update(cf v, cf f, cf a) {
+#pragma clang fp contract(off)
+    const float ii = f.im * a.im, ri = f.re * a.im;
+    const float tre = __builtin_fmaf(f.re, a.re, -ii);
+    const float tim = __builtin_fmaf(f.im, a.re, ri);
+    return cf{v.re - tre, v.im - tim};
+  }
+};
+template <class Sync = BlockSync, bool PIN = false>
+__device__ __forceinline__ void eliminate(cf* A, int lda, int N, int ncol, bool gj, cf* fac, int* piv, cf* logdet,
+                          int tid = threadIdx.x, int nt = blockDim.x, int width = 64, Sync sync = Sync{}) {
+  if (tid == 0) *logdet = cf{0.f, 0.f};
+  sync();
+  for (int p = 0; p < N; ++p) {
+    find_pivot(A, lda, N, p, piv, tid, width);
+    sync();
+    const int pr = *piv;
+    if (pr != p) {
+      for (int c = tid; c < ncol; c += nt) {
+        const cf t = A[p * lda + c];
+        A[p * lda + c] = A[pr * lda + c];
+        A[pr * lda + c] = t;
+      }
+    }
+    sync();
+    const cf P = A[p * lda + p];
+    if (tid == 0) {
+      const float mag = PIN ? sqrtf(PinnedLu::mag2(P)) : sqrtf(P.re * P.re + P.im * P.im);
+      logdet->re += logf(mag);
+      logdet->im += atan2f(P.im, P.re) + (pr != p ? kPi : 0.f);
+    }
+    const cf Pinv = cdiv(cf{1.f, 0.f}, P);
+    sync();
+    if (gj) {
+      for (int r = tid; r < N; r += nt) fac[r] = (r == p) ? cf{0.f, 0.f} : A[r * lda + p];
+      for (int c = tid; c < ncol; c += nt) A[p * lda + c] = A[p * lda + c] * Pinv;
+    } else {
+      for (int r = tid; r < N; r += nt)
+        fac[r] = (r > p) ? (PIN ? PinnedLu::factor(A[r * lda + p], Pinv) : A[r * lda + p] * Pinv) : cf{0.f, 0.f};
+    }
+    sync();
+    const int r0 = gj ? 0 : p + 1;
+    const int c0 = gj ? 0 : p;
+    const int nr = N - r0, nc = ncol - c0;
+    for (int idx = tid; idx < nr * nc; idx += nt) {
+      const int r = r0 + idx / nc, c = c0 + idx % nc;
+      if (r == p) continue;
+      const cf f = fac[r];
+      cf v = A[r * lda + c];
+      const cf a = A[p * lda + c];
+      if constexpr (PIN) {
+        v = PinnedLu::update(v, f, a);
+      } else {
+        v.re -= f.re * a.re - f.im * a.im;
+        v.im -= f.re * a.im + f.im * a.re;
+      }
+      A[r * lda + c] = v;
+    }
+    sync();
+  }
+}
+
+template <int NMAX>
+__device__ __forceinline__ cf lu_logdet_cols(cf (&col)[NMAX], int N, int lane, int width) {
+  auto is = [](int r, int q) __attribute__((always_inline)) {
+    int m = r == q;
+    asm volatile("" : "+v"(m));
+    return m != 0;
+  };
+  auto pick = [&](int q) __attribute__((always_inline)) {
+    cf v = col[0];
+#pragma unroll
+    for (int r = 1; r < NMAX; ++r)
+      if (is(r, q)) v = col[r];
+    return v;
+  };
+  float lre = 0.f, lim = 0.f;
+  for (int p = 0; p < N; ++p) {
+    float best = -1.f;
+    int bi = N;
+#pragma unroll
+    for (int r = 0; r < NMAX; ++r) {
+      if (r >= p && r < N) {
+        const float v = cabs1(col[r]);
+        if (v > best) {
+          best = v;
+          bi = r;
+        }
+      }
+    }
+    int pr = __shfl(bi, p, width);
+    pr = pr < N ? pr : p;
+    if (pr != p) {
+      const cf a = pick(p), b = pick(pr);
+#pragma unroll
+      for (int r = 0; r < NMAX; ++r) {
+        if (is(r, p)) col[r] = b;
+        if (is(r, pr)) col[r] = a;
+      }
+    }
+    const cf mine = pick(p);
+    const cf P{__shfl(mine.re, p, width), __shfl(mine.im, p, width)};
+    const float mag = sqrtf(P.re * P.re + P.im * P.im);
+    lre += logf(mag);
+    lim += atan2f(P.im, P.re) + (pr != p ? kPi : 0.f);
+    const cf Pinv = cdiv(cf{1.f, 0.f}, P);
+#pragma unroll
+    for (int r = 0; r < NMAX; ++r) {
+      if (r > p && r < N) {
+#pragma clang fp contract(off)
+        const cf c = col[r];
+        const cf fl{c.re * Pinv.re - c.im * Pinv.im, __builtin_fmaf(c.im, Pinv.re, c.re * Pinv.im)};
+        const cf f{__shfl(fl.re, p, width), __shfl(fl.im, p, width)};
+        if (lane >= p) {
+          const float tre = __builtin_fmaf(f.re, mine.re, -(f.im * mine.im));
+          const float tim = __builtin_fmaf(f.im, mine.re, f.re * mine.im);
+          col[r] = cf{c.re - tre, c.im - tim};
+        }
+      }
+    }
+  }
+  return cf{lre, lim};
+}
+
+__device__ inline double jastrow_pair(double r, double al, double cst, double* f1, double* f2) {
+  const double ar = al + r;
+  *f1 = (cst * al * al) / (ar * ar);
+  *f2 = -2.0 * (cst * al * al) / (ar * ar * ar);
+  return -(cst * al * al) / ar;
+}
+
+template <int MGV, bool HW, class Sync, class FRows>
+__device__ __forceinline__ void det_value_body(float* sm_raw, FRows frow, const float* x,
+                                               const float* __restrict__ jas, const float* __restrict__ norm,
+                                               float* __restrict__ logpsi, int N, int n_up, int M, int K, int bw,
+                                               int nw, int tid, const McmcEpi& epi, Sync sync) {
+  static_assert(!HW || MGV == 0, "half-wave form: serial contraction only");
+  cf* E0 = reinterpret_cast<cf*>(sm_raw);
+  cf* A = E0 + N * M;
+  cf* fac = A + N * N;
+  cf* ld = fac + N;
+  cf* logdet = ld + K;
+  int* piv = reinterpret_cast<int*>(logdet + 1);
+  const bool live = bw < nw;
+  const int b = live ? bw : nw - 1;
+  const int nt = HW ? 32 : 64, width = HW ? 32 : 64;
+  double* cart = reinterpret_cast<double*>(piv + 2);
+  DET_T(0, 0);
+  for (int idx = tid; idx < N * M; idx += nt) {
+    const int i = idx / M, p = idx % M;
+    E0[idx] = env_leaf(x[2 * (b * N + i)], x[2 * (b * N + i) + 1], p, M, norm[p], false, 0.f, true).e0;
+  }
+  for (int i = tid; i < N; i += nt) {
+    double st, ct, sp, cp;
+    sincos((double)x[2 * (b * N + i)], &st, &ct);
+    sincos((double)x[2 * (b * N + i) + 1], &sp, &cp);
+    cart[3 * i] = st * cp;
+    cart[3 * i + 1] = st * sp;
+    cart[3 * i + 2] = ct;
+  }
+  sync();
+  DET_T(0, 1);
+  double Jw = 0.0;
+  {
+    const double ap = jas[0], aa = jas[1];
+    for (int q = tid; q < N * N; q += nt) {
+      const int i = q / N, j = q - (q / N) * N;
+      if (j <= i) continue;
+      const double dx = cart[3 * j] - cart[3 * i], dy = cart[3 * j + 1] - cart[3 * i + 1],
+                   dz = cart[3 * j + 2] - cart[3 * i + 2];
+      const double r = sqrt(dx * dx + dy * dy + dz * dz);
+      const bool same = (i < n_up) == (j < n_up);
+      double f1, f2;
+      Jw += jastrow_pair(r, same ? ap : aa, same ? 0.25 : 0.5, &f1, &f2);
+    }
+    for (int o = width >> 1; o > 0; o >>= 1) Jw += __shfl_xor(Jw, o, width);
+  }
+  DET_T(0, 2);
+  const int G = 64 / N, gj = tid % N, gg = tid / N, NK = N * K, MNK = M * NK;
+  for (int k = 0; k < K; ++k) {
+    if constexpr (MGV == 0) {
+      for (int idx = tid; idx < N * N; idx += nt) {
+        const int i = idx / N, j = idx % N;
+        const int blk = (i >= n_up && n_up > 0) ? 1 : 0;
+        const float* rp = frow(b, i) + (size_t)blk * 2 * MNK + (size_t)j * K + k;
+        cf acc{0.f, 0.f};
+        for (int p0 = 0; p0 < M; p0 += 16) {
+          float fr[16], fi[16];
+#pragma unroll
+          for (int q = 0; q < 16; ++q) {
+            const size_t p = (size_t)min(p0 + q, M - 1);
+            fr[q] = rp[p * NK];
+            fi[q] = rp[(size_t)MNK + p * NK];
+          }
+#pragma unroll
+          for (int q = 0; q < 16; ++q)
+            if (p0 + q < M) cfma(acc, cf{fr[q], fi[q]}, E0[i * M + p0 + q]);
+        }
+        A[idx] = acc;
+      }
+    }
+    if constexpr (MGV > 0) {
+      constexpr int NF = 2 * (MGV > 0 ? MGV : 1);
+      auto ldrow = [&](int i, float (&f)[NF]) __attribute__((always_inline)) {
+        const int blk = (i >= n_up && n_up > 0) ? 1 : 0;
+        const float* rp = frow(b, i) + (size_t)blk * 2 * MNK + (size_t)gj * K + k;
+#pragma unroll
+        for (int u = 0; u < MGV; ++u) {
+          const size_t m = (size_t)min(gg + G * u, M - 1);
+          f[2 * u] = rp[m * NK];
+          f[2 * u + 1] = rp[(size_t)MNK + m * NK];
+        }
+      };
+      auto contract = [&](int i, const float (&f)[NF]) __attribute__((always_inline)) {
+        cf acc{0.f, 0.f};
+#pragma unroll
+        for (int u = 0; u < MGV; ++u) {
+          const int m = gg + G * u;
+          const bool ok = gg < G && m < M;
+          cfma(acc, cf{ok ? f[2 * u] : 0.f, ok ? f[2 * u + 1] : 0.f}, E0[i * M + min(m, M - 1)]);
+        }
+        float re = acc.re, im = acc.im;
+        for (int q = 1; q < G; ++q) {
+          re += __shfl(acc.re, gj + N * q, 64);
+          im += __shfl(acc.im, gj + N * q, 64);
+        }
+        if (gg == 0) A[i * N + gj] = cf{re, im};
+      };
+      float fa[NF], fb[NF];
+      if constexpr (MGV <= 24) {
+        ldrow(0, fa);
+        for (int i = 0; i < N; i += 2) {
+          ldrow(min(i + 1, N - 1), fb);
+          contract(i, fa);
+          ldrow(min(i + 2, N - 1), fa);
+          if (i + 1 < N) contract(i + 1, fb);
+        }
+      } else {
+        for (int i = 0; i < N; ++i) {
+          ldrow(i, fa);
+          contract(i, fa);
+        }
+      }
+    }
+    sync();
+    DET_T(0, 3);
+    if (N <= 8 && DET_LU_REG) {
+      cf col[8];
+#pragma unroll
+      for (int r = 0; r < 8; ++r) col[r] = (r < N && tid < N) ? A[r * N + tid] : cf{0.f, 0.f};
+      const cf l = lu_logdet_cols<8>(col, N, tid, width);
+      if (tid == 0) ld[k] = l;
+    } else {
+      eliminate<Sync, HW>(A, N, N, N, false, fac, piv, logdet, tid, nt, width, sync);
+      if (tid == 0) ld[k] = *logdet;
+    }
+    sync();
+    DET_T(0, 4);
+  }
+  float* lpv = reinterpret_cast<float*>(cart + 3 * N);
+  if (tid == 0 && live) {
+    float lmax = -INFINITY;
+    for (int k = 0; k < K; ++k) lmax = fmaxf(lmax, ld[k].re);
+    float zr = 0.f, zi = 0.f;
+    for (int k = 0; k < K; ++k) {
+      const float mag = expf(ld[k].re - lmax);
+      zr += mag * cosf(ld[k].im);
+      zi += mag * sinf(ld[k].im);
+    }
+    float val_re = 0.5f * logf(zr * zr + zi * zi) + lmax;
+    float val_im = atan2f(zi, zr);
+    logpsi[2 * b] = val_re + (float)Jw;
+    logpsi[2 * b + 1] = val_im;
+    *lpv = val_re + (float)Jw;
+  }
+  DET_T(0, 5);
+  if (!epi.on) return;
+  sync();
+  if (!live || tid >= N) return;
+  const float lp2 = 2.f * *lpv;
+  const bool cond = accept_one(lp2, epi.lp[b], b, N, epi.seed, epi.step, epi.woff, epi.noise);
+  const int e = b * N + tid;
+  float th = epi.x[2 * e], ph = epi.x[2 * e + 1];
+  if (cond) {
+    th = x[2 * e];
+    ph = x[2 * e + 1];
+    epi.x[2 * e] = th;
+    epi.x[2 * e + 1] = ph;
+    if (tid == 0) {
+      epi.lp[b] = lp2;
+      epi.nacc[b] += 1;
+    }
+  }
+  if (epi.propose)
+    propose_one(th, ph, epi.x2, epi.geo, e, b, tid, N, epi.width, epi.seed, epi.step + 1, epi.woff, epi.noise2);
+  DET_T(0, 6);
+}
+
+}
diff --git a/deephall_amd/csrc/dh_internal.h b/deephall_amd/csrc/dh_internal.h
--- a/deephall_amd/csrc/dh_internal.h
+++ b/deephall_amd/csrc/dh_internal.h
@@ -82,11 +82,28 @@
   int qkv_gemm;
   int orbital;
   int det;
+  int det_in_chain;
 };
 constexpr int kTrunkRouteFields = 12;
-static_assert(sizeof(TrunkRoute) == kTrunkRouteFields * sizeof(int), "dh_debug_route copies the fields as ints");
+static_assert(sizeof(TrunkRoute) == (kTrunkRouteFields + 1) * sizeof(int) &&
+                  offsetof(TrunkRoute, det_in_chain) == kTrunkRouteFields * sizeof(int),
+              "dh_debug_route copies the first kTrunkRouteFields fields as ints");
 int gemm_family(const Dims& d, bool want_x6);
 TrunkRoute trunk_route(const Dims& d, int gemm_mode, int C, int rows);
+int set_det_in_chain(int on);
+
+constexpr int kChainTileRows = 96;
+constexpr size_t kChainPlaneBytes = 3 * (size_t)kChainTileRows * 264 * 2;
+inline int det_value_per(const Dims& d) {
+  return (2 * d.N * d.M + 2 * d.N * d.N + 2 * d.N + 2 * d.K + 2 + 4 + 6 * d.N + 2 + 3 + 1) & ~3;
+}
+inline bool det_value_half_wave(const Dims& d) {
+  const int mgv = (d.M + 64 / d.N - 1) / (64 / d.N);
+  return mgv <= 2 && d.N * d.N <= 64;
+}
+inline int det_chain_ldf(const Dims& d) {
+  return d.orb_cols + (((d.N * d.K - d.orb_cols) % 32) + 32) % 32;
+}
 
 constexpr int kRowPad = 256;
 constexpr int kWalkerRowPad = 768;
@@ -151,10 +168,11 @@
 void launch_l1_basis(const Dims& d, const float* W0, const float* UT, const float* bol, const float* ln1,
                      const float* Wm, const float* bm, float* BT, float* VT, hipStream_t s);
 bool chain_attn_supported(int N, int H, int dh);
+struct ChainDet;
 void launch_chain_x6(const float* X1, const uint16_t* Wp1, int ldp1, const float* b1, const float* ln1,
                      const uint16_t* Wp2, int ldp2, const float* b2, const float* ln2, const uint16_t* Wp3, int ldp3,
                      const float* b3, int n3, float* Y3, int ldy3, float* h, int rows, X6Feat feat, hipStream_t s,
-                     bool store_h = true);
+                     bool store_h = true, const ChainDet* det = nullptr, bool store_F = true);
 void launch_transpose(const float* src, int ld_src, int rows, int cols, float* dst, int ld_dst, hipStream_t s);
 
 void launch_input(const Dims& d, const float* x, const float* W0, const float* W0qkv, const float* bqkv, float* h,
@@ -199,6 +217,16 @@
 };
 void launch_det_value(const Dims& d, const float* F, const float* x, const float* jastrow, const float* norm,
                       float* logpsi, int nw, hipStream_t s, const McmcEpi& epi = McmcEpi{});
+struct ChainDet {
+  const float* x = nullptr;
+  const float* jastrow = nullptr;
+  const float* norm = nullptr;
+  float* logpsi = nullptr;
+  int N = 0, n_up = 0, M = 0, K = 0, nw = 0;
+  int per = 0;
+  int ldf = 0;
+  McmcEpi epi;
+};
 void launch_histograms(const float* x, int B, int N, int db, int pb, float* dens, float* pair, hipStream_t s);
 void launch_monopole_orbitals(const float* pts, int n, int flux, float* out, hipStream_t s);
 bool det_precontract(const Dims& d);
diff --git a/deephall_amd/csrc/gemm_x6.hip b/deephall_amd/csrc/gemm_x6.hip
--- a/deephall_amd/csrc/gemm_x6.hip
+++ b/deephall_amd/csrc/gemm_x6.hip
@@ -4,6 +4,7 @@
 #include "attn_val.h"
 #include "dh_internal.h"
 #include "device_common.h"
+#include "det_value.h"
 
 #ifndef CHAIN_STAMP
 #define CHAIN_STAMP 0
@@ -1024,12 +1025,15 @@
   int rows;
   X6Feat feat;
   int store_h;
+  int store_F;
+  ChainDet det;
 };
 
 constexpr int CS_NW = 8, CS_RB = CH_BM / 32, CS_PD = 4, CS_LSP = 264;
 constexpr int CS_PRMF = 5 * 256;
 constexpr size_t CS_PLANE = (size_t)CH_BM * CS_LSP * 2, CS_SMEM = 3 * CS_PLANE + 2 * CS_NW * CH_BM * 4 + CS_PRMF * 4;
 static_assert(CS_SMEM <= 163840, "chain LDS");
+static_assert(CH_BM == kChainTileRows && 3 * CS_PLANE == kChainPlaneBytes, "trunk_route's LDS bound of the determinant tail");
 
 __device__ __forceinline__ void split4(const float4& x, uint2& h, uint2& m, uint2& l) {
   const float a[4] = {x.x, x.y, x.z, x.w};
@@ -1049,8 +1053,11 @@
   l = make_uint2(Lv[0], Lv[1]);
 }
 
-template <int NA = 0>
+constexpr int kChainDet = -1;
+template <int NAT = 0>
 __global__ __launch_bounds__(512) void chain_x6s_kernel(ChainArgs a) {
+  constexpr bool DET = NAT == kChainDet;
+  constexpr int NA = DET ? 0 : NAT;
   constexpr int RB = CS_RB, PD = CS_PD, LSP = CS_LSP;
   using K16 = std::integral_constant<int, CH_K / 16>;
   using KP1 = std::integral_constant<int, (NA > 0 ? CH_KO / 16 : CH_K / 16)>;
@@ -1517,6 +1524,54 @@
   if (!a.Wp3) return;
   lbar();
   CHAIN_T(9);
+  if constexpr (DET) {
+    const bool mine = 32 * wid < a.n3;
+    if (mine) gemm(Tr{}, K16{}, Zero{});
+    CHAIN_T(10);
+    lbar();
+    float* Ft = reinterpret_cast<float*>(smem);
+    int tl;
+    asm volatile("v_mbcnt_lo_u32_b32 %0, -1, 0\n\tv_mbcnt_hi_u32_b32 %0, -1, %0" : "=v"(tl));
+    const int t32 = tl & 31, th = tl >> 5;
+    using KArg = const __attribute__((address_space(4))) char;
+    KArg* kp = (KArg*)__builtin_amdgcn_kernarg_segment_ptr();
+    asm volatile("" : "+s"(kp));
+    const ChainDet det = *(const ChainDet*)(kp + offsetof(ChainArgs, det));
+    const int ldf = det.ldf;
+    if (mine) {
+      const int c = 32 * wid + t32;
+      const bool cok = c < a.n3;
+      const float bv = cok ? a.b3[c] : 0.f;
+      if (cok) {
+        float* fc = Ft + 4 * th * ldf + c;
+#pragma unroll
+        for (int rb = 0; rb < RB; ++rb) {
+#pragma unroll
+          for (int q = 0; q < 16; ++q) fc[(32 * rb + (q & 3) + 8 * (q >> 2)) * ldf] = acc[rb][q] + bv;
+        }
+      }
+    }
+    lbar();
+    CHAIN_T(11);
+    if (a.store_F) {
+      const int nrow = min(CH_BM, rows - row0);
+      for (int i = 64 * wid + tl; i < nrow * a.n3; i += 512) {
+        const int r = i / a.n3, c = i - r * a.n3;
+        a.Y3[(size_t)(row0 + r) * a.ldy3 + c] = Ft[r * ldf + c];
+      }
+    }
+    const int N = det.N, WT = CH_BM / N, w0 = bid * WT;
+    float* reg = Ft + CH_BM * ldf + (2 * wid + th) * det.per;
+    for (int pr = wid; 2 * pr < WT; pr += CS_NW) {
+      const int bw0 = w0 + 2 * pr;
+      if (bw0 >= det.nw) break;
+      WaveSync{}();
+      det_value_body<0, true>(reg, FRowsTile{Ft, ldf, N, w0}, det.x, det.jastrow, det.norm, det.logpsi, N, det.n_up,
+                              det.M, det.K, bw0 + th, det.nw, t32, det.epi, WaveSync{});
+    }
+    CHAIN_T(12);
+    return;
+  }
   for (int col0 = 0; col0 < a.n3; col0 += CH_BN) {
     if (col0 + 32 * wid >= a.n3) continue;
     gemm(Tr{}, K16{}, Zero{});
@@ -1550,7 +1605,6 @@
     if (col0 < 3 * CH_BN) CHAIN_T(11 + 2 * (col0 / CH_BN));
   }
 }
-
 
 }
 
@@ -1688,9 +1742,11 @@
 void launch_chain_x6(const float* X1, const uint16_t* Wp1, int ldp1, const float* b1, const float* ln1,
                      const uint16_t* Wp2, int ldp2, const float* b2, const float* ln2, const uint16_t* Wp3, int ldp3,
                      const float* b3, int n3, float* Y3, int ldy3, float* h, int rows, X6Feat feat, hipStream_t s,
-                     bool store_h) {
-  ChainArgs a{X1, Wp1, Wp2, Wp3, ldp1, ldp2, ldp3, b1, ln1, b2, ln2, b3, n3, ldy3, Y3, h, rows, feat, store_h ? 1 : 0};
+                     bool store_h, const ChainDet* det, bool store_F) {
+  ChainArgs a{X1, Wp1, Wp2, Wp3, ldp1, ldp2, ldp3, b1, ln1, b2, ln2, b3, n3, ldy3, Y3, h, rows, feat, store_h ? 1 : 0,
+              store_F ? 1 : 0, det ? *det : ChainDet{}};
   auto k = chain_x6s_kernel<0>;
+  if (det) k = chain_x6s_kernel<kChainDet>;
   if (feat.W0qkv) {
     switch (feat.N) {
       case 2: k = chain_x6s_kernel<2>; break;
diff --git a/deephall_amd/csrc/trunk_route.cpp b/deephall_amd/csrc/trunk_route.cpp
--- a/deephall_amd/csrc/trunk_route.cpp
+++ b/deephall_amd/csrc/trunk_route.cpp
@@ -1,6 +1,13 @@
+#include <atomic>
+
 #include "dh_internal.h"
 
 namespace dh {
+
+namespace {
+std::atomic<int> g_det_in_chain{1};
+}
+int set_det_in_chain(int on) { return g_det_in_chain.exchange(on ? 1 : 0); }
 
 int gemm_family(const Dims& d, bool want_x6) {
   const bool nt = d.D % 32 == 0;
@@ -45,6 +52,10 @@
   }
   r.input_h = !r.h0_epilogue;
   r.input_skip = !channels && r.h0_epilogue;
+  const int last_form = d.L > 1 ? r.form1 : r.form0;
+  r.det_in_chain = g_det_in_chain.load() && !channels && d.L > 0 && last_form == LF_CHAIN && r.orbital == ORB_IN_CHAIN &&
+                   det_value_half_wave(d) && kChainTileRows % d.N == 0 && d.orb_cols <= 256 &&
+                   (size_t)kChainTileRows * det_chain_ldf(d) * 4 + 16 * (size_t)det_value_per(d) * 4 <= kChainPlaneBytes;
   return r;
 }
 
diff --git a/include/deephall_amd.h b/include/deephall_amd.h
--- a/include/deephall_amd.h
+++ b/include/deephall_amd.h
@@ -172,6 +172,8 @@
 
 int dh_debug_gemm_x6_choice(int rows, int ncols);
 int dh_debug_route(const dh_handle* h, int B, int op, int* out, int n);
+int dh_debug_set_det_in_chain(int on);
+int dh_debug_det_in_chain(const dh_handle* h, int B, int op);
 int dh_debug_x6_plane_rows(int ncols);
 int dh_debug_split_planes(const float* Wt, int ldw, int ncols, int K, uint16_t* Wp, void* stream);
 int dh_debug_gemm_x6(int variant, const float* X, int ldx, const uint16_t* Wp, int ldp, const float* bias,
```
